# Arthur151/ROMP

Measured on AMD Instinct MI355X. Metric: images/sec (512x512, HRNet-32), higher is better.
Workload: dtype f32 (convs as f16x2-split products, f32 accumulate; same 1e-4 parity gate as f32 MFMA); 1 GPU; ROMP HRNet-32 512x512, batch=1024 synthetic images sharded across 1 GPU (BASELINE configs[2]), each shard walked in forward calls of batch=32 (BASELINE configs[1]); net+parse+SMPL per call; batch_per_call=32, global_batch=1024, hipgraph=True, autotune=True, variant_table=committed romp_amd/tune/romp_hrnet32_f16x2_b32.json, branch_streams=True, conv_math=f16x2, parallelism=dp1, cross_step_pipeline=True, rccl_ranks=1, backend=none (single process)

## Files before the change

### __graft_entry__.py

```python
import os
import sys

ROOT = os.path.dirname(os.path.abspath(__file__))
if ROOT not in sys.path:
    sys.path.insert(0, ROOT)


def build():
    import subprocess
    from romp_amd import build as b
    path = b.build(force=False)
    assert os.path.exists(path)
    import romp_amd
    from romp_amd import lib
    h = lib.load()
    for name in lib.EXPORTS + lib.VIEW_EXPORTS:
        assert hasattr(h, name), name
    from oracle import romp_oracle
    if os.path.isdir('/root/reference/simple_romp/vis_human/sim3drender/lib'):
        subprocess.run(['make', '-C', os.path.join(ROOT, 'oracle')], check=True, stdout=subprocess.DEVNULL)
        from oracle import sim3dr_oracle, ref_cpu
        assert sim3dr_oracle.load_ref() is not None
        assert ref_cpu.available() and ref_cpu.bev_available(), 'oracle/_ref/{romp,bev}/*.pyc missing'
    print('built', path, 'abi', h.romp_abi_version())


def smoke():
    import numpy as np
    import torch
    assert torch.cuda.is_available(), 'smoke() needs the MI355X'
    import romp_amd
    from oracle import romp_oracle as O
    settings = romp_amd.romp_settings([])
    settings.GPU, settings.center_thresh, settings.max_batch = 0, 1.3, 2
    sd = O.make_romp_state_dict(0, center_bias=2.0)
    smpl = O.make_synthetic_smpl(0)
    model = romp_amd.ROMP(settings, state_dict=sd, smpl_model=smpl)
    img = O.make_images(1, seed=3)
    out, bids = model.forward_batch(img.to('cuda:0'))
    torch.cuda.synchronize()
    cm, pm = O.romp_net_forward(sd, img)
    ref = O.parsing_outputs(cm.numpy(), pm.numpy(), settings.center_thresh)
    assert out is not None and ref is not None
    assert np.array_equal(out['center_preds'].cpu().numpy(), ref['center_preds']), 'detections differ'
    th = out['smpl_thetas'].cpu().numpy()
    vo, jo, _ = O.smpl_forward(smpl, out['smpl_betas'].cpu().numpy(), th)
    ev = float(np.abs(out['verts'].cpu().numpy() - vo).max())
    et = float(np.abs(th - ref['smpl_thetas']).max())
    print(f'smoke: {len(ref["batch_ids"])} persons, verts max-abs vs oracle {ev:.2e}, thetas {et:.2e}')
    assert ev < 1e-4, ev
    assert et < 1e-3, et


if __name__ == '__main__':
    build()
    if len(sys.argv) > 1 and sys.argv[1] == 'smoke':
        smoke()
```

### romp_amd/build.py

```python
import concurrent.futures as cf
import os
import subprocess
import sys

HERE = os.path.dirname(os.path.abspath(__file__))
CSRC = os.path.join(HERE, 'csrc')
LIB = os.path.join(HERE, 'libromp_hip.so')
SOURCES = ['conv_h2.hip', 'conv_h2c.hip', 'conv_h2c32.hip', 'conv_f32.hip', 'conv_h2d.hip', 'conv_h2b.hip', 'conv_h2r.hip',
           'conv_h2s.hip', 'conv_mfma.hip', 'conv_h2k.hip', 'conv_h2g.hip', 'conv_h2x.hip', 'conv_fup.hip', 'stem_fuse.hip', 'stem2.hip', 'stem7p.hip', 'net.hip', 'parse.hip', 'smpl.hip', 'bev.hip',
           'post.hip', 'crowd.hip', 'render.hip', 'temporal.hip']
OPTIONAL_BX3 = 'conv_bx3.hip'
_UNROLL = ['-mllvm', '-pragma-unroll-threshold=1000000']
EXTRA_FLAGS = {'conv_h2b.hip': _UNROLL, 'conv_h2c.hip': _UNROLL, 'conv_h2c32.hip': _UNROLL}
FLAGS = ['--offload-arch=gfx950', '-O3', '-std=c++17', '-fPIC', '-Wall', '-Wno-unused-function', '-Wno-unused-value', '-Wno-unused-result']


def _hipcc():
    for c in (os.environ.get('HIPCC'), '/opt/rocm/bin/hipcc', 'hipcc'):
        if c and (os.path.isabs(c) and os.path.exists(c) or not os.path.isabs(c)):
            return c
    raise RuntimeError('hipcc not found')


def _stale(target, deps):
    if not os.path.exists(target):
        return True
    t = os.path.getmtime(target)
    return any(os.path.getmtime(d) > t for d in deps)


def build(force=False, verbose=False, extra_flags=(), lib=None, objdir=None, with_bx3=None):
    hipcc = _hipcc()
    if with_bx3 is None:
        with_bx3 = os.environ.get('ROMP_WITH_BX3', '0') not in ('', '0')
    sources = SOURCES + ([OPTIONAL_BX3] if with_bx3 else [])
    headers = [os.path.join(CSRC, f) for f in os.listdir(CSRC) if f.endswith('.h')] + \
              [os.path.join(HERE, '..', 'include', h) for h in ('romp_hip.h', 'romp_hip_views.h')]
    objdir = objdir or os.path.join(HERE, 'build')
    lib = lib or LIB
    os.makedirs(objdir, exist_ok=True)
    jobs = []
    for s in sources:
        src = os.path.join(CSRC, s)
        obj = os.path.join(objdir, s.replace('.hip', '.o'))
        if force or _stale(obj, [src] + headers):
            jobs.append((src, obj))

    def cc(job):
        src, obj = job
        cmd = [hipcc] + FLAGS + list(extra_flags) + EXTRA_FLAGS.get(os.path.basename(src), []) + ['-c', src, '-o', obj]
        r = subprocess.run(cmd, capture_output=True, text=True)
        if r.returncode != 0:
            raise RuntimeError('hipcc failed for %s:\n%s' % (src, r.stderr[-4000:]))
        if verbose and r.stderr.strip():
            print(r.stderr, file=sys.stderr)
        return obj

    with cf.ThreadPoolExecutor(max_workers=min(8, max(1, len(jobs)))) as ex:
        list(ex.map(cc, jobs))
    objs = [os.path.join(objdir, s.replace('.hip', '.o')) for s in sources]
    marker = os.path.join(objdir, '.with_bx3')
    relink = os.path.exists(marker) != bool(with_bx3)
    if force or jobs or relink or _stale(lib, objs):
        cmd = [hipcc, '--offload-arch=gfx950', '-shared', '-fPIC'] + objs + ['-o', lib]
        r = subprocess.run(cmd, capture_output=True, text=True)
        if r.returncode != 0:
            raise RuntimeError('link failed:\n' + r.stderr[-4000:])
        if with_bx3:
            open(marker, 'w').close()
        elif os.path.exists(marker):
            os.remove(marker)
    return lib


if __name__ == '__main__':
    print(build(force='--force' in sys.argv, verbose=True))
```

### romp_amd/csrc/common.h

```cpp
#pragma once
#include <hip/hip_runtime.h>
#include <stdint.h>
#include <stdio.h>
#include <stdarg.h>
#include "../../include/romp_hip.h"

namespace romp {

void set_error(const char* fmt, ...);

#define ROMP_HIP_CHECK(expr)                                                          \
    do {                                                                              \
        hipError_t _e = (expr);                                                       \
        if (_e != hipSuccess) {                                                       \
            romp::set_error("%s failed: %s (%s:%d)", #expr, hipGetErrorString(_e),    \
                            __FILE__, __LINE__);                                      \
            return ROMP_EHIP;                                                         \
        }                                                                             \
    } while (0)

#define ROMP_REQUIRE(cond, ...)                                                       \
    do {                                                                              \
        if (!(cond)) {                                                                \
            romp::set_error(__VA_ARGS__);                                             \
            return ROMP_EINVAL;                                                       \
        }                                                                             \
    } while (0)

constexpr int QUEUE_STRIDE = 32, QUEUE_INTS = 8 * QUEUE_STRIDE;

int launch_conv(const romp_op& op, const float* in, const float* res, float* out, int B,
                int mode, int variant, int* queue, hipStream_t st, int wg_cap = 0);
int describe_conv(const romp_op& op, int B, int variant, char* out, int n);
int conv_num_variants();
int conv_family_variants(int math);
int conv_trace_read(unsigned long long* dst_host, int max_words);
int conv_init();
bool conv_variant_valid(const romp_op& op, int variant);
bool conv_variant_tunable(const romp_op& op, int variant);
void conv_set_sat_counter(int* counter, bool checked_fused);
int* conv_sat_counter();
void conv_set_wg_cap(int cap);
int conv_wg_cap();
bool conv_sat_checked();
unsigned long long* conv_trace_arm(hipStream_t st);
int launch_seam1x1(const romp_op& opa, const romp_op& opb, const romp_op* opd, const float* m, const float* x, float* t, float* u, int B, hipStream_t st);
int launch_bblock32r(const romp_op& op1, const romp_op& op2, const float* x, float* y, int B, int* queue, hipStream_t st);
int launch_bblock64(const romp_op& op1, const romp_op& op2, const float* x, float* y, int B, int* queue, hipStream_t st);
int launch_bblock32(const romp_op& op1, const romp_op& op2, const float* x, float* y, int B, int* queue, hipStream_t st);
int launch_stem(const romp_op& op, const float* image, float* out, int B, hipStream_t st);
int launch_stem7(const romp_op& op, const float* image, float* out, int B, hipStream_t st);
int launch_stem2(const romp_op& stem, const romp_op& op, const float* image, float* out, int B, hipStream_t st);
int launch_maxpool(const romp_op& op, const float* in, float* out, int B, hipStream_t st);
int launch_stem7p(const romp_op& op, const float* image, float* out, int B, hipStream_t st);
struct FuseTerm { const float* ptr; int shift; int cstride; int fmt; };
int launch_fusesum(const FuseTerm* terms, int n_terms, float* out, int B, int H, int W, int C,
                   int out_cstride, int out_coff, int relu, hipStream_t st, int out_fmt = 0, int act_shift = 0);

int launch_fuseup(const romp_op& op, const FuseTerm* terms, float* out, int B, hipStream_t st);

int launch_ksum(const romp_op& op, const float* partial, const float* res, float* out, int B, hipStream_t st);

int launch_bev_pack(const float* fv, int fv_cs, const float* feats, int f_cs, float* out, int B, hipStream_t st);
int launch_bev_maps(const float* fv, int fv_cs, const float* bv, int bv_cs, const float* anchors_host, float* center3d,
                    float* cam3d, int B, hipStream_t st);
int launch_conv3d(int C, const float* w_host, const float* scale_host, const float* shift_host, int relu, const float* in,
                  const float* res, float* out, int B, hipStream_t st);

}
```

### romp_amd/csrc/parse.hip

```cpp
#include "common.h"
#include "rot6d.h"
#include <vector>

#pragma clang fp contract(off)

namespace romp {

constexpr int MAP = 64, NPIX = MAP * MAP;

constexpr int PARSE_THREADS = 1024;
__global__ __launch_bounds__(PARSE_THREADS) void parse_nms_topk_kernel(const float* __restrict__ center, float thresh,
                                                              int max_person, int32_t* __restrict__ ws) {
    __shared__ float s_map[NPIX];
    __shared__ float s_score[NPIX];
    __shared__ int s_idx[NPIX];
    __shared__ int s_count;
    const int b = blockIdx.x, tid = threadIdx.x;
    const float* cm = center + (size_t)b * NPIX;
    for (int p = tid; p < NPIX; p += PARSE_THREADS) s_map[p] = cm[p];
    if (tid == 0) s_count = 0;
    __syncthreads();
    for (int p = tid; p < NPIX; p += PARSE_THREADS) {
        const int y = p / MAP, x = p % MAP;
        const float v = s_map[p];
        float m = v;
        for (int dy = -2; dy <= 2; ++dy) {
            const int yy = y + dy;
            if ((unsigned)yy >= (unsigned)MAP) continue;
            for (int dx = -2; dx <= 2; ++dx) {
                const int xx = x + dx;
                if ((unsigned)xx >= (unsigned)MAP) continue;
                m = fmaxf(m, s_map[yy * MAP + xx]);
            }
        }
        const float score = (m == v) ? v : v * 0.0f;
        if (score > thresh) {
            const int slot = atomicAdd(&s_count, 1);
            s_score[slot] = score;
            s_idx[slot] = p;
        }
    }
    __syncthreads();
    const int n = s_count;
    int32_t* w = ws + (size_t)b * (2 * max_person + 2);
    for (int c = tid; c < n; c += PARSE_THREADS) {
        const float sc = s_score[c];
        const int id = s_idx[c];
        int rank = 0;
        for (int k = 0; k < n; ++k) {
            const float so = s_score[k];
            rank += (so > sc) || (so == sc && s_idx[k] < id);
        }
        if (rank < max_person) {
            w[rank] = id;
            w[max_person + rank] = __float_as_int(sc);
        }
    }
    if (tid == 0) {
        w[2 * max_person] = n < max_person ? n : max_person;
        w[2 * max_person + 1] = n;
    }
}

__global__ __launch_bounds__(64) void parse_pack_kernel(
    const float* __restrict__ center, const float* __restrict__ params, int B, int max_person,
    int32_t* __restrict__ ws, int32_t* batch_ids, int32_t* flat_inds, float* scores, float* params_pred,
    float* cam, float* thetas, float* betas, int32_t* center_preds, const int32_t* watch) {
    const int r = blockIdx.x, b = blockIdx.y, lane = threadIdx.x;
    const int stride = 2 * max_person + 2;
    if (watch && r == 0 && b == 0 && lane == 0)
        ws[(size_t)B * stride] = __hip_atomic_load(watch, __ATOMIC_RELAXED, __HIP_MEMORY_SCOPE_AGENT);
    const int cnt = ws[(size_t)b * stride + 2 * max_person];
    if (r >= cnt) return;
    int off = 0;
    for (int k = lane; k < b; k += 64) off += ws[(size_t)k * stride + 2 * max_person];
    for (int d = 32; d > 0; d >>= 1) off += __shfl_xor(off, d);
    const int row = off + r;
    const int flat = ws[(size_t)b * stride + r];
    const float sc = __int_as_float(ws[(size_t)b * stride + max_person + r]);
    __shared__ float s_p[148];
    const float* src = params + ((size_t)b * NPIX + flat) * 145;
    for (int c = lane; c < 145; c += 64) {
        float v = src[c];
        if (c == 0) v = powf(1.1f, v);
        s_p[c] = v;
        params_pred[(size_t)row * 145 + c] = v;
    }
    __syncthreads();
    if (lane < 3) cam[row * 3 + lane] = s_p[lane];
    if (lane < 10) betas[row * 10 + lane] = s_p[135 + lane];
    if (lane < 22) {
        float aa[3];
        rot6d_to_aa_dev(s_p + 3 + lane * 6, aa);
        thetas[row * 72 + lane * 3 + 0] = aa[0];
        thetas[row * 72 + lane * 3 + 1] = aa[1];
        thetas[row * 72 + lane * 3 + 2] = aa[2];
    } else if (lane < 28) {
        thetas[row * 72 + 66 + (lane - 22)] = 0.f;
    }
    if (lane == 0) {
        batch_ids[row] = b;
        flat_inds[row] = flat;
        scores[row] = sc;
        center_preds[row * 2 + 0] = (flat % MAP) * 512 / 64;
        center_preds[row * 2 + 1] = (flat / MAP) * 512 / 64;
    }
}

__global__ void rot6d_kernel(const float* __restrict__ x6, int n, float* __restrict__ aa) {
    const int i = blockIdx.x * blockDim.x + threadIdx.x;
    if (i >= n) return;
    float x[6], o[3];
    for (int k = 0; k < 6; ++k) x[k] = x6[(size_t)i * 6 + k];
    rot6d_to_aa_dev(x, o);
    for (int k = 0; k < 3; ++k) aa[(size_t)i * 3 + k] = o[k];
}

__global__ void project_kernel(const float* __restrict__ joints, int N, int J, const float* __restrict__ cam,
                               float pad_size, float left, float top, float* pj2d, float* pj2d_org,
                               float* cam_trans) {
    const int i = blockIdx.x * blockDim.x + threadIdx.x;
    if (i < N * J) {
        const int n = i / J;
        const float s = cam[n * 3], tx = cam[n * 3 + 1], ty = cam[n * 3 + 2];
        const float px = joints[(size_t)i * 3] * s + tx, py = joints[(size_t)i * 3 + 1] * s + ty;
        pj2d[(size_t)i * 2] = px; pj2d[(size_t)i * 2 + 1] = py;
        pj2d_org[(size_t)i * 2] = (px + 1.f) * pad_size / 2.f - left;
        pj2d_org[(size_t)i * 2 + 1] = (py + 1.f) * pad_size / 2.f - top;
    }
    if (i < N) {
        const float s = cam[i * 3], tx = cam[i * 3 + 1], ty = cam[i * 3 + 2];
        cam_trans[i * 3 + 0] = (tx / s) * 2.f;
        cam_trans[i * 3 + 1] = (ty / s) * 2.f;
        cam_trans[i * 3 + 2] = (1.f / s) * 2.f;
    }
}

__global__ void cam_to_trans_kernel(const float* __restrict__ cam, int N, float weight, float* __restrict__ trans) {
    const int i = blockIdx.x * blockDim.x + threadIdx.x;
    if (i >= N) return;
    const float s = cam[i * 3], tx = cam[i * 3 + 1], ty = cam[i * 3 + 2];
    trans[i * 3 + 0] = (tx / s) * weight;
    trans[i * 3 + 1] = (ty / s) * weight;
    trans[i * 3 + 2] = (1.f / s) * weight;
}

__global__ __launch_bounds__(64) void translation_lsq_kernel(const float* __restrict__ joints, int J, int K, const float* __restrict__ pj2d,
                                                               double f, double cx, double cy, float* __restrict__ trans) {
    const int n = blockIdx.x, lane = threadIdx.x;
    double a02 = 0, a12 = 0, a22 = 0, b0 = 0, b1 = 0, b2 = 0;
    int cnt = 0;
    for (int k = lane; k < K; k += 64) {
        const float* X = joints + ((size_t)n * J + k) * 3;
        const float uf = (pj2d[((size_t)n * J + k) * 2] + 1.f) * (float)cx, vf = (pj2d[((size_t)n * J + k) * 2 + 1] + 1.f) * (float)cy;
        if (!(vf > -2.f) || X[2] == -2.f) continue;
        ++cnt;
        const double u = uf, v = vf;
        const double qx = cx - u, qy = cy - v;
        const double rx = (u - cx) * (double)X[2] - f * (double)X[0], ry = (v - cy) * (double)X[2] - f * (double)X[1];
        a02 += f * qx; a12 += f * qy; a22 += qx * qx + qy * qy;
        b0 += f * rx; b1 += f * ry; b2 += qx * rx + qy * ry;
    }
    for (int d = 32; d > 0; d >>= 1) {
        a02 += __shfl_xor(a02, d); a12 += __shfl_xor(a12, d); a22 += __shfl_xor(a22, d);
        b0 += __shfl_xor(b0, d); b1 += __shfl_xor(b1, d); b2 += __shfl_xor(b2, d);
        cnt += __shfl_xor(cnt, d);
    }
    if (lane == 0) {
        const double d = (double)cnt * f * f;
        const double piv = a22 - (a02 * a02 + a12 * a12) / d;
        float t0 = -1.f, t1 = -1.f, t2 = -1.f;
        if (cnt >= 4 && fabs(piv) > 1e-12 * fabs(a22)) {
            const double z = (b2 - (a02 * b0 + a12 * b1) / d) / piv;
            t0 = (float)((b0 - a02 * z) / d); t1 = (float)((b1 - a12 * z) / d); t2 = (float)z;
        }
        trans[n * 3] = t0; trans[n * 3 + 1] = t1; trans[n * 3 + 2] = t2;
    }
}

#pragma clang fp contract(off)
__global__ void project_verts_kernel(const float* __restrict__ verts, size_t total, int V, const float* __restrict__ cam,
                                     float pad_size, float left, float top, float* __restrict__ camed, float* __restrict__ org) {
    const size_t i = blockIdx.x * (size_t)blockDim.x + threadIdx.x;
    if (i >= total) return;
    const size_t n = i / V;
    const float s = cam[n * 3], tx = cam[n * 3 + 1], ty = cam[n * 3 + 2];
    const float px = verts[i * 3] * s + tx, py = verts[i * 3 + 1] * s + ty, pz = verts[i * 3 + 2];
    if (camed) { camed[i * 3] = px; camed[i * 3 + 1] = py; camed[i * 3 + 2] = pz; }
    org[i * 3] = (px + 1.f) * pad_size / 2.f - left;
    org[i * 3 + 1] = (py + 1.f) * pad_size / 2.f - top;
    org[i * 3 + 2] = (pz + 1.f) * pad_size / 2.f;
}

__global__ void bev_project_verts_kernel(const float* __restrict__ verts, size_t total, int V, const float* __restrict__ trans,
                                         float pad_size, float left, float top, float* __restrict__ org) {
    const size_t i = blockIdx.x * (size_t)blockDim.x + threadIdx.x;
    if (i >= total) return;
    const size_t n = i / V;
    const float vz = verts[i * 3 + 2];
    const float x = verts[i * 3] + trans[n * 3], y = verts[i * 3 + 1] + trans[n * 3 + 1], z = vz + trans[n * 3 + 2] + 1e-6f;
    const float px = x / z * 443.4f / 256.f, py = y / z * 443.4f / 256.f;
    org[i * 3] = (px + 1.f) * pad_size / 2.f - left;
    org[i * 3 + 1] = (py + 1.f) * pad_size / 2.f - top;
    org[i * 3 + 2] = (vz + 1.f) * pad_size / 2.f;
}

}

using namespace romp;

extern "C" {

int romp_bev_project_verts(const float* verts, int N, int V, const float* cam_trans, const float* pad_info_host, float* verts_camed_org,
                           void* stream) {
    ROMP_REQUIRE(verts && cam_trans && pad_info_host && verts_camed_org && N > 0 && V > 0, "romp_bev_project_verts: bad arguments");
    const float top = pad_info_host[0], left = pad_info_host[2], h = pad_info_host[4], w = pad_info_host[5];
    const size_t total = (size_t)N * V;
    hipLaunchKernelGGL(bev_project_verts_kernel, dim3((unsigned)((total + 255) / 256)), dim3(256), 0, (hipStream_t)stream, verts, total,
                       V, cam_trans, h > w ? h : w, left, top, verts_camed_org);
    ROMP_HIP_CHECK(hipGetLastError());
    return ROMP_OK;
}

int romp_project_verts(const float* verts, int N, int V, const float* cam, const float* pad_info_host, float* verts_camed,
                       float* verts_camed_org, void* stream) {
    ROMP_REQUIRE(verts && cam && pad_info_host && verts_camed_org && N > 0 && V > 0, "romp_project_verts: bad arguments");
    const float top = pad_info_host[0], left = pad_info_host[2], h = pad_info_host[4], w = pad_info_host[5];
    const size_t total = (size_t)N * V;
    hipLaunchKernelGGL(project_verts_kernel, dim3((unsigned)((total + 255) / 256)), dim3(256), 0, (hipStream_t)stream, verts, total, V,
                       cam, h > w ? h : w, left, top, verts_camed, verts_camed_org);
    ROMP_HIP_CHECK(hipGetLastError());
    return ROMP_OK;
}

int romp_parse_watch(const float* center_maps, const float* params_maps, int B, float conf_thresh, int max_person,
                     int32_t* count_host, int32_t* batch_ids, int32_t* flat_inds, float* scores, float* params_pred,
                     float* cam, float* thetas, float* betas, int32_t* center_preds, int32_t* workspace, void* stream,
                     const int32_t* watch, int32_t* watch_host) {
    ROMP_REQUIRE(center_maps && params_maps && workspace && B > 0, "romp_parse: bad arguments");
    ROMP_REQUIRE(max_person >= 1 && max_person <= 1024, "romp_parse: max_person %d out of range", max_person);
    ROMP_REQUIRE(batch_ids && flat_inds && scores && params_pred && cam && thetas && betas && center_preds,
                 "romp_parse: null output");
    hipStream_t st = (hipStream_t)stream;
    hipLaunchKernelGGL(parse_nms_topk_kernel, dim3(B), dim3(PARSE_THREADS), 0, st, center_maps, conf_thresh, max_person, workspace);
    ROMP_HIP_CHECK(hipGetLastError());
    hipLaunchKernelGGL(parse_pack_kernel, dim3(max_person, B), dim3(64), 0, st, center_maps, params_maps, B, max_person,
                       workspace, batch_ids, flat_inds, scores, params_pred, cam, thetas, betas, center_preds, watch);
    ROMP_HIP_CHECK(hipGetLastError());
    if (!count_host) return ROMP_OK;
    const size_t n_cnt = (size_t)B * (2 * max_person + 2);
    std::vector<int32_t> cnt(n_cnt + 1);
    ROMP_HIP_CHECK(hipMemcpyAsync(cnt.data(), workspace, (n_cnt + (watch ? 1 : 0)) * sizeof(int32_t), hipMemcpyDeviceToHost, st));
    ROMP_HIP_CHECK(hipStreamSynchronize(st));
    int total = 0;
    for (int b = 0; b < B; ++b) total += cnt[(size_t)b * (2 * max_person + 2) + 2 * max_person];
    *count_host = total;
    if (watch && watch_host) *watch_host = cnt[n_cnt];
    return ROMP_OK;
}

int romp_parse(const float* center_maps, const float* params_maps, int B, float conf_thresh, int max_person,
               int32_t* count_host, int32_t* batch_ids, int32_t* flat_inds, float* scores, float* params_pred,
               float* cam, float* thetas, float* betas, int32_t* center_preds, int32_t* workspace, void* stream) {
    return romp_parse_watch(center_maps, params_maps, B, conf_thresh, max_person, count_host, batch_ids, flat_inds, scores, params_pred,
                            cam, thetas, betas, center_preds, workspace, stream, nullptr, nullptr);
}

int romp_rot6d_to_aa(const float* x6, int n, float* aa, void* stream) {
    ROMP_REQUIRE(x6 && aa && n >= 0, "romp_rot6d_to_aa: bad arguments");
    if (n == 0) return ROMP_OK;
    hipLaunchKernelGGL(rot6d_kernel, dim3((n + 127) / 128), dim3(128), 0, (hipStream_t)stream, x6, n, aa);
    ROMP_HIP_CHECK(hipGetLastError());
    return ROMP_OK;
}

int romp_cam_to_trans(const float* cam, int N, float weight, float* trans, void* stream) {
    ROMP_REQUIRE(cam && trans && N >= 0, "romp_cam_to_trans: bad arguments");
    if (N == 0) return ROMP_OK;
    hipLaunchKernelGGL(cam_to_trans_kernel, dim3((N + 255) / 256), dim3(256), 0, (hipStream_t)stream, cam, N, weight, trans);
    ROMP_HIP_CHECK(hipGetLastError());
    return ROMP_OK;
}

int romp_estimate_translation(const float* joints, int N, int J, int K, const float* pj2d, float focal_length, float img_size,
                              float* trans, void* stream) {
    ROMP_REQUIRE(joints && pj2d && trans && N >= 0 && J > 0 && K >= 2 && K <= J, "romp_estimate_translation: bad arguments");
    if (N == 0) return ROMP_OK;
    hipLaunchKernelGGL(translation_lsq_kernel, dim3(N), dim3(64), 0, (hipStream_t)stream, joints, J, K, pj2d, (double)focal_length,
                       (double)img_size / 2.0, (double)img_size / 2.0, trans);
    ROMP_HIP_CHECK(hipGetLastError());
    return ROMP_OK;
}

int romp_project(const float* joints, int N, int J, const float* cam, const float* pad_info_host, float* pj2d,
                 float* pj2d_org, float* cam_trans, void* stream) {
    ROMP_REQUIRE(joints && cam && pad_info_host && pj2d && pj2d_org && cam_trans && N >= 0 && J > 0,
                 "romp_project: bad arguments");
    if (N == 0) return ROMP_OK;
    const float top = pad_info_host[0], left = pad_info_host[2], h = pad_info_host[4], w = pad_info_host[5];
    const float pad_size = h > w ? h : w;
    const int total = N * J;
    hipLaunchKernelGGL(project_kernel, dim3((total + 255) / 256), dim3(256), 0, (hipStream_t)stream, joints, N, J, cam,
                       pad_size, left, top, pj2d, pj2d_org, cam_trans);
    ROMP_HIP_CHECK(hipGetLastError());
    return ROMP_OK;
}

}
```

### romp_amd/csrc/smpl.hip

```cpp
#include "common.h"
#include <vector>

namespace romp {

constexpr int NV = 6890, NJ = 24, NPF = 207, NJOUT = 71, NREG = 26, NPICK = 21;
constexpr int PB = 16;
constexpr int NT = (NV + 63) / 64;
constexpr int MAXLV = NJ;

typedef float f2 __attribute__((ext_vector_type(2)));
__device__ __forceinline__ f2 pk_fma(f2 a, f2 b, f2 c) { return __builtin_elementwise_fma(a, b, c); }

struct Parents { int p[NJ]; };
struct Levels { int n; int start[MAXLV + 1]; int order[NJ]; };

__global__ __launch_bounds__(256) void smpl_prep_kernel(const float* __restrict__ Jreg, const float* __restrict__ vt,
                                                         const float* __restrict__ sd, int nb, float* __restrict__ Jt,
                                                         float* __restrict__ Js) {
    const int j = blockIdx.x, e = blockIdx.y;
    const int k = e / (nb + 1), l = e % (nb + 1);
    double acc = 0.0;
    for (int v = threadIdx.x; v < NV; v += 256) {
        const float w = Jreg[(size_t)j * NV + v];
        const float x = (l == nb) ? vt[v * 3 + k] : sd[((size_t)v * 3 + k) * nb + l];
        acc += (double)w * (double)x;
    }
    __shared__ double s[256];
    s[threadIdx.x] = acc;
    __syncthreads();
    for (int d = 128; d > 0; d >>= 1) {
        if (threadIdx.x < d) s[threadIdx.x] += s[threadIdx.x + d];
        __syncthreads();
    }
    if (threadIdx.x == 0) {
        if (l == nb) Jt[j * 3 + k] = (float)s[0];
        else Js[(j * 3 + k) * nb + l] = (float)s[0];
    }
}

template <int NB>
__global__ __launch_bounds__(64) void smpl_pose_kernel(const float* __restrict__ betas,
                                                        const float* __restrict__ thetas,
                                                        const float* __restrict__ Jt, const float* __restrict__ Js,
                                                        const int* __restrict__ sched, float* __restrict__ pose_feat,
                                                        float* __restrict__ Amat, float* __restrict__ joints) {
    __shared__ float sR[NJ][9], sJ[NJ][3], sG[NJ][12];
    const int n = blockIdx.x, lane = threadIdx.x;
    if (lane < NJ) {
        const float* r = thetas + (size_t)n * 72 + lane * 3;
        const float rx0 = r[0], ry0 = r[1], rz0 = r[2];
        float jt[3], js[3][NB], bt[NB];
#pragma unroll
        for (int l = 0; l < NB; ++l) bt[l] = betas[(size_t)n * NB + l];
#pragma unroll
        for (int k = 0; k < 3; ++k) {
            jt[k] = Jt[lane * 3 + k];
#pragma unroll
            for (int l = 0; l < NB; ++l) js[k][l] = Js[(lane * 3 + k) * NB + l];
        }
        const float ex = rx0 + 1e-8f, ey = ry0 + 1e-8f, ez = rz0 + 1e-8f;
        const float angle = sqrtf(ex * ex + ey * ey + ez * ez);
        const float rx = rx0 / angle, ry = ry0 / angle, rz = rz0 / angle;
        float sn, cs;
        sincosf(angle, &sn, &cs);
        const float oc = 1.f - cs;
        const float kk00 = -(rz * rz) - ry * ry, kk11 = -(rz * rz) - rx * rx, kk22 = -(ry * ry) - rx * rx;
        const float kk01 = ry * rx, kk02 = rz * rx, kk12 = rz * ry;
        float R[9];
        R[0] = 1.f + oc * kk00;      R[1] = sn * -rz + oc * kk01; R[2] = sn * ry + oc * kk02;
        R[3] = sn * rz + oc * kk01;  R[4] = 1.f + oc * kk11;      R[5] = sn * -rx + oc * kk12;
        R[6] = sn * -ry + oc * kk02; R[7] = sn * rx + oc * kk12;  R[8] = 1.f + oc * kk22;
#pragma unroll
        for (int e = 0; e < 9; ++e) sR[lane][e] = R[e];
        if (lane >= 1) {
            float* pf = pose_feat + (size_t)(n / PB) * NPF * PB + (n % PB);
#pragma unroll
            for (int e = 0; e < 9; ++e) pf[((lane - 1) * 9 + e) * PB] = R[e] - ((e == 0 || e == 4 || e == 8) ? 1.f : 0.f);
        }
#pragma unroll
        for (int k = 0; k < 3; ++k) {
            float a = jt[k];
#pragma unroll
            for (int l = 0; l < NB; ++l) a = fmaf(bt[l], js[k][l], a);
            sJ[lane][k] = a;
        }
    }
    __syncthreads();
    const int grp = lane / 12, el = lane % 12, rr = el / 4, cc = el % 4;
    if (lane < 12) sG[0][lane] = (cc < 3) ? sR[0][rr * 3 + cc] : sJ[0][rr];
    __syncthreads();
    const int n_lv = sched[0];
    for (int lv = 1; lv < n_lv; ++lv) {
        const int q1 = sched[1 + lv + 1];
        for (int q = sched[1 + lv] + grp; q < q1 && grp < 5; q += 5) {
            const int i = sched[1 + (MAXLV + 1) + q], p = sched[1 + (MAXLV + 1) + NJ + i];
            float v;
            if (cc < 3) {
                v = sG[p][rr * 4 + 0] * sR[i][0 * 3 + cc];
                v = fmaf(sG[p][rr * 4 + 1], sR[i][1 * 3 + cc], v);
                v = fmaf(sG[p][rr * 4 + 2], sR[i][2 * 3 + cc], v);
            } else {
                v = sG[p][rr * 4 + 0] * (sJ[i][0] - sJ[p][0]);
                v = fmaf(sG[p][rr * 4 + 1], sJ[i][1] - sJ[p][1], v);
                v = fmaf(sG[p][rr * 4 + 2], sJ[i][2] - sJ[p][2], v);
                v += sG[p][rr * 4 + 3];
            }
            sG[i][el] = v;
        }
        __syncthreads();
    }
    for (int idx = lane; idx < NJ * 12; idx += 64) {
        const int j = idx / 12, e = idx % 12, r = e / 4, c = e % 4;
        float v = sG[j][e];
        if (c == 3) {
            joints[((size_t)n * NJOUT + j) * 3 + r] = v;
            const float t = sG[j][r * 4 + 0] * sJ[j][0] + sG[j][r * 4 + 1] * sJ[j][1] + sG[j][r * 4 + 2] * sJ[j][2];
            v -= t;
        }
        Amat[(size_t)n * NJ * 12 + idx] = v;
    }
}

constexpr int SKIN_WAVES = 4, KQ = (NPF + SKIN_WAVES - 1) / SKIN_WAVES;
constexpr int PPW = PB / SKIN_WAVES;
constexpr int U_FLOATS = SKIN_WAVES * PB * 3 * 64;
constexpr int KC = 13, NCH = KQ / KC;
static_assert(KQ == KC * NCH, "chunking of the pose-blend quarter");

__device__ __forceinline__ void pd_load(float (&d)[KC][3], const float* __restrict__ pdv, int kbase) {
#pragma unroll
    for (int i = 0; i < KC; ++i) {
        const size_t off = (size_t)min(kbase + i, NPF - 1) * (NV * 3);
        d[i][0] = pdv[off]; d[i][1] = pdv[off + 1]; d[i][2] = pdv[off + 2];
    }
}

__device__ __forceinline__ void pd_blend(f2 (&po)[PB / 2][3], const float (&d)[KC][3], const float (*s_pf)[PB], int kbase) {
#pragma unroll
    for (int i = 0; i < KC; ++i) {
        const int k = kbase + i;
        const bool in = k < NPF;
        const float d0 = in ? d[i][0] : 0.f, d1 = in ? d[i][1] : 0.f, d2 = in ? d[i][2] : 0.f;
        const f2 dd0{d0, d0}, dd1{d1, d1}, dd2{d2, d2};
        const float* row = s_pf[min(k, NPF - 1)];
#pragma unroll
        for (int p4 = 0; p4 < PB; p4 += 4) {
            const float4 f = *reinterpret_cast<const float4*>(row + p4);
            const f2 fa{f.x, f.y}, fb{f.z, f.w};
            po[p4 / 2][0] = pk_fma(fa, dd0, po[p4 / 2][0]); po[p4 / 2][1] = pk_fma(fa, dd1, po[p4 / 2][1]); po[p4 / 2][2] = pk_fma(fa, dd2, po[p4 / 2][2]);
            po[p4 / 2 + 1][0] = pk_fma(fb, dd0, po[p4 / 2 + 1][0]); po[p4 / 2 + 1][1] = pk_fma(fb, dd1, po[p4 / 2 + 1][1]); po[p4 / 2 + 1][2] = pk_fma(fb, dd2, po[p4 / 2 + 1][2]);
        }
    }
}

constexpr int SVS = 196, RS = 68;
constexpr int RPAIRS = NREG / 2;
static_assert(NREG % 2 == 0 && PB * RPAIRS <= 256, "joint partials: one pass");
template <int NB>
__global__ __launch_bounds__(256) void smpl_skin_kernel(const float* __restrict__ betas, const float* __restrict__ pose_feat,
                                                         const float* __restrict__ Amat, const float* __restrict__ vt,
                                                         const float* __restrict__ sd, const float* __restrict__ pd,
                                                         const float* __restrict__ lbsw, const float* __restrict__ reg, int N, int groups,
                                                         float* __restrict__ verts, float* __restrict__ jpart) {
    __shared__ __attribute__((aligned(16))) float s_u[U_FLOATS];
    __shared__ __attribute__((aligned(16))) float s_A[5 * 256 * 4];
    __shared__ float s_beta[PB][NB];
    static_assert(NPF * PB <= U_FLOATS && 4 * 256 * 4 <= U_FLOATS && PB * SVS <= U_FLOATS && NREG * RS <= PB * NJ * 12 && NT % 4 == 0, "LDS aliasing");
    const int tid = threadIdx.x, lane = tid & 63, wave = tid >> 6;
    const int xcd = blockIdx.x & 7, slot = blockIdx.x >> 3;
    const int tile = (slot / groups) * 8 + xcd, grp = slot % groups;
    if (tile >= NT) return;
    const int p0 = grp * PB;
    const int np = min(PB, N - p0);
    const bool live = tile * 64 + lane < NV;
    const int v = min(tile * 64 + lane, NV - 1);
    const float* pdv = pd + (size_t)v * 3;
    const int k0 = wave * KQ;
    float d[2][KC][3];
    pd_load(d[0], pdv, k0);
    constexpr int PF4 = NPF * PB / 4, A4 = PB * NJ * 12 / 4;
    static_assert(PF4 <= 4 * 256 && A4 <= 5 * 256 && PB * NB <= 256, "staging loops");
    const float4* src_pf = reinterpret_cast<const float4*>(pose_feat + (size_t)grp * NPF * PB);
    const float4* src_A = reinterpret_cast<const float4*>(Amat + (size_t)p0 * NJ * 12);
    float4 tpf[4], tA[5];
#pragma unroll
    for (int i = 0; i < 4; ++i) tpf[i] = src_pf[min(tid + 256 * i, PF4 - 1)];
#pragma unroll
    for (int i = 0; i < 5; ++i) tA[i] = src_A[min(tid + 256 * i, A4 - 1)];
    const float tb = (tid < PB * NB && tid / NB < np) ? betas[(size_t)p0 * NB + tid] : 0.f;
#pragma unroll
    for (int i = 0; i < 4; ++i) reinterpret_cast<float4*>(s_u)[tid + 256 * i] = tpf[i];
#pragma unroll
    for (int i = 0; i < 5; ++i) reinterpret_cast<float4*>(s_A)[tid + 256 * i] = tA[i];
    if (tid < PB * NB) (&s_beta[0][0])[tid] = tb;
    __syncthreads();
    const float(*s_pf)[PB] = reinterpret_cast<const float(*)[PB]>(s_u);
    f2 po[PB / 2][3];
#pragma unroll
    for (int p = 0; p < PB / 2; ++p) po[p][0] = po[p][1] = po[p][2] = f2{0.f, 0.f};
#pragma unroll
    for (int c = 0; c < NCH; ++c) {
        if (c + 1 < NCH) pd_load(d[(c + 1) & 1], pdv, k0 + (c + 1) * KC);
        pd_blend(po, d[c & 1], s_pf, k0 + c * KC);
    }
    const float t0 = vt[v * 3 + 0], t1 = vt[v * 3 + 1], t2 = vt[v * 3 + 2];
    float sdv[3][NB];
#pragma unroll
    for (int k = 0; k < 3; ++k)
#pragma unroll
        for (int l = 0; l < NB; ++l) sdv[k][l] = sd[((size_t)v * 3 + k) * NB + l];
    f2 w[NJ];
#pragma unroll
    for (int j4 = 0; j4 < NJ; j4 += 4) {
        const float4 t = *reinterpret_cast<const float4*>(lbsw + (size_t)v * NJ + j4);
        w[j4] = f2{t.x, t.x}; w[j4 + 1] = f2{t.y, t.y}; w[j4 + 2] = f2{t.z, t.z}; w[j4 + 3] = f2{t.w, t.w};
    }
    float treg[7];
    static_assert(NREG * 64 <= 7 * 256, "regressor tile staging");
#pragma unroll
    for (int i = 0; i < 7; ++i) {
        const int idx = min(tid + 256 * i, NREG * 64 - 1), vv = tile * 64 + (idx & 63);
        const float x = reg[(size_t)(idx >> 6) * NV + min(vv, NV - 1)];
        treg[i] = vv < NV ? x : 0.f;
    }
    __syncthreads();
    float(*s_po)[PB * 3][64] = reinterpret_cast<float(*)[PB * 3][64]>(s_u);
#pragma unroll
    for (int p = 0; p < PB / 2; ++p)
#pragma unroll
        for (int k = 0; k < 3; ++k) {
            s_po[wave][(2 * p) * 3 + k][lane] = po[p][k].x;
            s_po[wave][(2 * p + 1) * 3 + k][lane] = po[p][k].y;
        }
    __syncthreads();
    float out[PPW][3];
#pragma unroll
    for (int pp = 0; pp < PPW; ++pp) {
        const int p = wave * PPW + pp;
        float a0 = 0.f, a1 = 0.f, a2 = 0.f;
#pragma unroll
        for (int l = 0; l < NB; ++l) {
            const float bb = s_beta[p][l];
            a0 = fmaf(bb, sdv[0][l], a0); a1 = fmaf(bb, sdv[1][l], a1); a2 = fmaf(bb, sdv[2][l], a2);
        }
        float q[3];
#pragma unroll
        for (int k = 0; k < 3; ++k)
            q[k] = (s_po[0][p * 3 + k][lane] + s_po[1][p * 3 + k][lane]) + (s_po[2][p * 3 + k][lane] + s_po[3][p * 3 + k][lane]);
        const float x = q[0] + (t0 + a0), y = q[1] + (t1 + a1), z = q[2] + (t2 + a2);
        f2 T[6];
#pragma unroll
        for (int e = 0; e < 6; ++e) T[e] = f2{0.f, 0.f};
        const float* Ap = s_A + p * NJ * 12;
#pragma unroll
        for (int j = 0; j < NJ; ++j) {
            const float4 a0v = *reinterpret_cast<const float4*>(Ap + j * 12);
            const float4 a1v = *reinterpret_cast<const float4*>(Ap + j * 12 + 4);
            const float4 a2v = *reinterpret_cast<const float4*>(Ap + j * 12 + 8);
            T[0] = pk_fma(w[j], f2{a0v.x, a0v.y}, T[0]); T[1] = pk_fma(w[j], f2{a0v.z, a0v.w}, T[1]);
            T[2] = pk_fma(w[j], f2{a1v.x, a1v.y}, T[2]); T[3] = pk_fma(w[j], f2{a1v.z, a1v.w}, T[3]);
            T[4] = pk_fma(w[j], f2{a2v.x, a2v.y}, T[4]); T[5] = pk_fma(w[j], f2{a2v.z, a2v.w}, T[5]);
        }
        out[pp][0] = fmaf(T[0].x, x, fmaf(T[0].y, y, fmaf(T[1].x, z, T[1].y)));
        out[pp][1] = fmaf(T[2].x, x, fmaf(T[2].y, y, fmaf(T[3].x, z, T[3].y)));
        out[pp][2] = fmaf(T[4].x, x, fmaf(T[4].y, y, fmaf(T[5].x, z, T[5].y)));
        if (live && p < np) {
            float* o = verts + ((size_t)(p0 + p) * NV + v) * 3;
            o[0] = out[pp][0]; o[1] = out[pp][1]; o[2] = out[pp][2];
        }
    }
    __syncthreads();
#pragma unroll
    for (int pp = 0; pp < PPW; ++pp)
#pragma unroll
        for (int k = 0; k < 3; ++k) s_u[(wave * PPW + pp) * SVS + k * 64 + lane] = out[pp][k];
#pragma unroll
    for (int i = 0; i < 7; ++i) {
        const int idx = tid + 256 * i;
        if (idx < NREG * 64) s_A[(idx >> 6) * RS + (idx & 63)] = treg[i];
    }
    __syncthreads();
    if (tid < PB * RPAIRS) {
        const int p = tid % PB, rp = tid / PB;
        const float* sv = s_u + p * SVS;
        const float* sr = s_A + rp * 2 * RS;
        f2 acc[3] = {f2{0.f, 0.f}, f2{0.f, 0.f}, f2{0.f, 0.f}};
#pragma unroll 4
        for (int i = 0; i < 64; i += 4) {
            const float4 x4 = *reinterpret_cast<const float4*>(sv + i), y4 = *reinterpret_cast<const float4*>(sv + 64 + i),
                         z4 = *reinterpret_cast<const float4*>(sv + 128 + i);
            const float4 r0 = *reinterpret_cast<const float4*>(sr + i), r1 = *reinterpret_cast<const float4*>(sr + RS + i);
#define JSTEP(c)                                                             \
            acc[0] = pk_fma(f2{r0.c, r1.c}, f2{x4.c, x4.c}, acc[0]);        \
            acc[1] = pk_fma(f2{r0.c, r1.c}, f2{y4.c, y4.c}, acc[1]);        \
            acc[2] = pk_fma(f2{r0.c, r1.c}, f2{z4.c, z4.c}, acc[2]);
            JSTEP(x) JSTEP(y) JSTEP(z) JSTEP(w)
#undef JSTEP
        }
        if (p < np) {
            float* o = jpart + (((size_t)(p0 + p) * NT + tile) * NREG + rp * 2) * 3;
            o[0] = acc[0].x; o[1] = acc[1].x; o[2] = acc[2].x;
            o[3] = acc[0].y; o[4] = acc[1].y; o[5] = acc[2].y;
        }
    }
}

__global__ __launch_bounds__(256) void smpl_joints_kernel(const float* __restrict__ verts, const float* __restrict__ jpart,
                                                           const int* __restrict__ pick, int root_align, float* __restrict__ joints,
                                                           float* __restrict__ root) {
    __shared__ float s_j[NJOUT * 3];
    const int n = blockIdx.x, tid = threadIdx.x;
    const float* vn = verts + (size_t)n * NV * 3;
    float* jn = joints + (size_t)n * NJOUT * 3;
    __shared__ float s_part[3][NREG * 3];
    static_assert(NT % 3 == 0 && 3 * NREG * 3 <= 256 && NREG * 3 + NPICK * 3 + NJ * 3 <= 256, "thread roles");
    if (tid < 3 * NREG * 3) {
        const int e = tid % (NREG * 3), part = tid / (NREG * 3);
        const float* src = jpart + ((size_t)n * NT + part * (NT / 3)) * NREG * 3 + e;
        float t[NT / 3];
#pragma unroll
        for (int u = 0; u < NT / 3; ++u) t[u] = src[(size_t)u * NREG * 3];
        float acc[4] = {0.f, 0.f, 0.f, 0.f};
#pragma unroll
        for (int u = 0; u < NT / 3; ++u) acc[u & 3] += t[u];
        s_part[part][e] = (acc[0] + acc[1]) + (acc[2] + acc[3]);
    }
    __syncthreads();
    if (tid < NREG * 3) {
        s_j[(NJ + NPICK) * 3 + tid] = (s_part[0][tid] + s_part[1][tid]) + s_part[2][tid];
    } else if (tid < NREG * 3 + NPICK * 3) {
        const int e = tid - NREG * 3;
        s_j[NJ * 3 + e] = vn[pick[e / 3] * 3 + e % 3];
    } else if (tid < NREG * 3 + NPICK * 3 + NJ * 3) {
        const int e = tid - NREG * 3 - NPICK * 3;
        s_j[e] = jn[e];
    }
    __syncthreads();
    if (tid < NJOUT * 3) {
        float v = s_j[tid];
        if (root_align) {
            const float r0 = (s_j[45 * 3 + tid % 3] + s_j[46 * 3 + tid % 3]) / 2.f;
            v -= r0;
            if (tid < 3) root[n * 3 + tid] = r0;
        }
        if (root_align || tid >= NJ * 3) jn[tid] = v;
    }
}

__global__ __launch_bounds__(256) void smpl_root_sub_kernel(float* __restrict__ verts, const float* __restrict__ root) {
    const int n = blockIdx.y, i = blockIdx.x * 256 + threadIdx.x;
    static_assert(NV * 3 % 2 == 0, "person stride is a whole number of float2");
    if (i >= NV * 3 / 2) return;
    const float r0 = root[n * 3], r1 = root[n * 3 + 1], r2 = root[n * 3 + 2];
    float2* p = reinterpret_cast<float2*>(verts + (size_t)n * NV * 3) + i;
    float2 t = *p;
    const int c = (i * 2) % 3;
    t.x -= c == 0 ? r0 : (c == 1 ? r1 : r2);
    t.y -= c == 0 ? r1 : (c == 1 ? r2 : r0);
    *p = t;
}

}

using namespace romp;

struct smpl_ctx {
    int nb = 10;
    int cap = 0;
    Parents par;
    int* sched = nullptr;
    float* jpart = nullptr;
    float *vt = nullptr, *sd = nullptr, *pd = nullptr, *lbsw = nullptr, *reg = nullptr, *Jt = nullptr, *Js = nullptr;
    int* pick = nullptr;
    float *pose_feat = nullptr, *Amat = nullptr, *root = nullptr;
};

static int smpl_reserve(smpl_ctx* c, int N, hipStream_t st) {
    if (N <= c->cap) return ROMP_OK;
    if (c->pose_feat) hipFree(c->pose_feat);
    if (c->Amat) hipFree(c->Amat);
    if (c->root) hipFree(c->root);
    if (c->jpart) hipFree(c->jpart);
    c->pose_feat = c->Amat = c->root = c->jpart = nullptr;
    c->cap = 0;
    const size_t cap = (size_t)(N + PB - 1) / PB * PB;
    ROMP_HIP_CHECK(hipMalloc((void**)&c->pose_feat, cap * NPF * 4));
    ROMP_HIP_CHECK(hipMalloc((void**)&c->Amat, cap * NJ * 12 * 4));
    ROMP_HIP_CHECK(hipMalloc((void**)&c->root, cap * 3 * 4));
    ROMP_HIP_CHECK(hipMalloc((void**)&c->jpart, cap * NT * NREG * 3 * 4));
    ROMP_HIP_CHECK(hipMemsetAsync(c->pose_feat, 0, cap * NPF * 4, st));
    ROMP_HIP_CHECK(hipMemsetAsync(c->Amat, 0, cap * NJ * 12 * 4, st));
    c->cap = (int)cap;
    return ROMP_OK;
}

extern "C" {

int smpl_ctx_create(smpl_ctx** out, const float* v_template, const float* shapedirs, int n_betas,
                    const float* posedirs, const float* J_regressor, const float* lbs_weights,
                    const int64_t* parents_host, const float* J_regressor_extra9, const float* J_regressor_h36m17,
                    const int64_t* extra_idx_host, int max_persons, void* stream) {
    ROMP_REQUIRE(out && v_template && shapedirs && posedirs && J_regressor && lbs_weights && parents_host &&
                 J_regressor_extra9 && J_regressor_h36m17 && extra_idx_host, "smpl_ctx_create: null argument");
    ROMP_REQUIRE(n_betas == 10 || n_betas == 11, "smpl_ctx_create: n_betas %d (10 = SMPL, 11 = SMPL-A)", n_betas);
    hipStream_t st = (hipStream_t)stream;
    smpl_ctx* c = new smpl_ctx();
    c->nb = n_betas;
    for (int j = 0; j < NJ; ++j) {
        c->par.p[j] = (int)parents_host[j];
        if (j > 0 && (c->par.p[j] < 0 || c->par.p[j] >= j)) {
            set_error("smpl_ctx_create: parents[%d]=%d is not an earlier joint", j, c->par.p[j]);
            delete c;
            return ROMP_EINVAL;
        }
    }
    int sched_h[1 + (MAXLV + 1) + 2 * NJ] = {0}, depth[NJ] = {0}, n_lv = 1;
    for (int j = 1; j < NJ; ++j) {
        depth[j] = depth[c->par.p[j]] + 1;
        if (depth[j] + 1 > n_lv) n_lv = depth[j] + 1;
    }
    sched_h[0] = n_lv;
    for (int lv = 0, q = 0; lv < n_lv; ++lv) {
        sched_h[1 + lv] = q;
        for (int j = 0; j < NJ; ++j)
            if (depth[j] == lv) sched_h[1 + (MAXLV + 1) + q++] = j;
        sched_h[1 + lv + 1] = q;
    }
    for (int j = 0; j < NJ; ++j) sched_h[1 + (MAXLV + 1) + NJ + j] = j ? c->par.p[j] : 0;
    int pick_h[NPICK];
    for (int i = 0; i < NPICK; ++i) {
        pick_h[i] = (int)extra_idx_host[i];
        if (pick_h[i] < 0 || pick_h[i] >= NV) { set_error("smpl_ctx_create: extra index out of range"); delete c; return ROMP_EINVAL; }
    }
#define SMPL_ALLOC_COPY(dst, src, count)                                                           \
    do {                                                                                           \
        if (hipMalloc((void**)&(dst), (size_t)(count) * 4) != hipSuccess ||                        \
            hipMemcpyAsync((dst), (src), (size_t)(count) * 4, hipMemcpyDeviceToDevice, st) != hipSuccess) { \
            set_error("smpl_ctx_create: alloc/copy of " #dst " failed");                           \
            smpl_ctx_destroy(c);                                                                   \
            return ROMP_EHIP;                                                                      \
        }                                                                                          \
    } while (0)
    SMPL_ALLOC_COPY(c->vt, v_template, NV * 3);
    SMPL_ALLOC_COPY(c->sd, shapedirs, (size_t)NV * 3 * n_betas);
    SMPL_ALLOC_COPY(c->pd, posedirs, (size_t)NPF * NV * 3);
    SMPL_ALLOC_COPY(c->lbsw, lbs_weights, (size_t)NV * NJ);
#undef SMPL_ALLOC_COPY
    if (hipMalloc((void**)&c->reg, (size_t)NREG * NV * 4) != hipSuccess || hipMalloc((void**)&c->Jt, NJ * 3 * 4) != hipSuccess ||
        hipMalloc((void**)&c->Js, (size_t)NJ * 3 * n_betas * 4) != hipSuccess || hipMalloc((void**)&c->pick, NPICK * 4) != hipSuccess ||
        hipMalloc((void**)&c->sched, sizeof(sched_h)) != hipSuccess) {
        set_error("smpl_ctx_create: hipMalloc failed");
        smpl_ctx_destroy(c);
        return ROMP_ENOMEM;
    }
    hipMemcpyAsync(c->reg, J_regressor_extra9, (size_t)9 * NV * 4, hipMemcpyDeviceToDevice, st);
    hipMemcpyAsync(c->reg + (size_t)9 * NV, J_regressor_h36m17, (size_t)17 * NV * 4, hipMemcpyDeviceToDevice, st);
    hipMemcpyAsync(c->pick, pick_h, NPICK * 4, hipMemcpyHostToDevice, st);
    hipMemcpyAsync(c->sched, sched_h, sizeof(sched_h), hipMemcpyHostToDevice, st);
    hipLaunchKernelGGL(smpl_prep_kernel, dim3(NJ, 3 * (n_betas + 1)), dim3(256), 0, st, J_regressor, c->vt, c->sd, n_betas,
                       c->Jt, c->Js);
    if (hipStreamSynchronize(st) != hipSuccess || hipGetLastError() != hipSuccess) {
        set_error("smpl_ctx_create: constant preparation failed");
        smpl_ctx_destroy(c);
        return ROMP_EHIP;
    }
    int rc = smpl_reserve(c, max_persons > 0 ? max_persons : 64, st);
    if (rc) { smpl_ctx_destroy(c); return rc; }
    if (hipStreamSynchronize(st) != hipSuccess) {
        set_error("smpl_ctx_create: clearing the staging buffers failed");
        smpl_ctx_destroy(c);
        return ROMP_EHIP;
    }
    *out = c;
    return ROMP_OK;
}

int smpl_forward(smpl_ctx* c, const float* betas, int n_betas, const float* thetas, int N, int root_align,
                 float* verts, float* joints, void* stream) {
    ROMP_REQUIRE(c && betas && thetas && verts && joints && N >= 0, "smpl_forward: bad arguments");
    ROMP_REQUIRE(n_betas == c->nb, "smpl_forward: n_betas %d but context was built with %d", n_betas, c->nb);
    if (N == 0) return ROMP_OK;
    hipStream_t st = (hipStream_t)stream;
    int rc = smpl_reserve(c, N, st);
    if (rc) return rc;
    if (c->nb == 10)
        hipLaunchKernelGGL(smpl_pose_kernel<10>, dim3(N), dim3(64), 0, st, betas, thetas, c->Jt, c->Js, c->sched, c->pose_feat, c->Amat, joints);
    else
        hipLaunchKernelGGL(smpl_pose_kernel<11>, dim3(N), dim3(64), 0, st, betas, thetas, c->Jt, c->Js, c->sched, c->pose_feat, c->Amat, joints);
    ROMP_HIP_CHECK(hipGetLastError());
    const int groups = (N + PB - 1) / PB;
    const dim3 grid(8 * ((NT + 7) / 8) * groups);
    if (c->nb == 10)
        hipLaunchKernelGGL(smpl_skin_kernel<10>, grid, dim3(256), 0, st, betas, c->pose_feat, c->Amat, c->vt, c->sd, c->pd,
                           c->lbsw, c->reg, N, groups, verts, c->jpart);
    else
        hipLaunchKernelGGL(smpl_skin_kernel<11>, grid, dim3(256), 0, st, betas, c->pose_feat, c->Amat, c->vt, c->sd, c->pd,
                           c->lbsw, c->reg, N, groups, verts, c->jpart);
    ROMP_HIP_CHECK(hipGetLastError());
    hipLaunchKernelGGL(smpl_joints_kernel, dim3(N), dim3(256), 0, st, verts, c->jpart, c->pick, root_align, joints, c->root);
    ROMP_HIP_CHECK(hipGetLastError());
    if (root_align) {
        hipLaunchKernelGGL(smpl_root_sub_kernel, dim3((NV * 3 / 2 + 255) / 256, N), dim3(256), 0, st, verts, c->root);
        ROMP_HIP_CHECK(hipGetLastError());
    }
    return ROMP_OK;
}

void smpl_ctx_destroy(smpl_ctx* c) {
    if (!c) return;
    float* ptrs[] = {c->vt, c->sd, c->pd, c->lbsw, c->reg, c->Jt, c->Js, c->pose_feat, c->Amat, c->root, c->jpart};
    for (float* p : ptrs)
        if (p) hipFree(p);
    if (c->pick) hipFree(c->pick);
    if (c->sched) hipFree(c->sched);
    delete c;
}

}
```

### romp_amd/distributed.py

```python
import torch
import torch.distributed as dist

RECORD_BASE = 88


def shard_range(n_items, rank, world_size):
    base, rem = divmod(n_items, world_size)
    lo = rank * base + min(rank, rem)
    return lo, lo + base + (1 if rank < rem else 0)


def pack_records(outputs, batch_ids, img_offset, flat_inds=None, with_joints=False, with_verts=False):
    if outputs is None:
        return None
    N = outputs['cam'].shape[0]
    dev = outputs['cam'].device
    flat = flat_inds if flat_inds is not None else (outputs['center_preds'][:, 1] // 8 * 64 + outputs['center_preds'][:, 0] // 8)
    cols = [(batch_ids + img_offset).float().view(N, 1), flat.float().view(N, 1), outputs['center_confs'].view(N, 1),
            outputs['cam'], outputs['smpl_thetas'], outputs['smpl_betas']]
    if with_joints:
        cols.append(outputs['joints'].reshape(N, -1))
    if with_verts:
        cols.append(outputs['verts'].reshape(N, -1))
    return torch.cat([c.to(dev).float() for c in cols], 1).contiguous()


def record_width(with_joints=False, with_verts=False):
    return RECORD_BASE + (213 if with_joints else 0) + (6890 * 3 if with_verts else 0)


def all_gather_records(local, width, device, group=None, state=None):
    world = dist.get_world_size(group)
    n_local = 0 if local is None else local.shape[0]
    if state is not None and state.get('cap', 0) > 0:
        cap = state['cap']
        block = torch.zeros(cap + 1, width, device=device, dtype=torch.float32)
        block[0, 0] = float(n_local)
        if n_local:
            block[1:1 + min(n_local, cap)] = local[:cap]
        gathered = torch.empty(world * (cap + 1), width, device=device, dtype=torch.float32)
        _all_gather_block(gathered, block, world, device, group)
        counts = [int(v) for v in gathered.view(world, cap + 1, width)[:, 0, 0].tolist()]
        if max(counts) <= cap:
            state['exchanges'] = state.get('exchanges', 0) + 1
            parts = [gathered[r * (cap + 1) + 1: r * (cap + 1) + 1 + counts[r]] for r in range(world)]
            return (torch.cat(parts, 0) if sum(counts) else torch.zeros(0, width, device=device)), counts
        state['cap'] = _capacity(max(counts))
        state['regrown'] = state.get('regrown', 0) + 1
        return all_gather_records(local, width, device, group, state)
    counts = [torch.zeros(1, dtype=torch.int64, device=device) for _ in range(world)]
    dist.all_gather(counts, torch.tensor([n_local], dtype=torch.int64, device=device), group=group)
    counts = torch.cat(counts).tolist()
    n_max = max(counts)
    if state is not None:
        state['cap'] = _capacity(n_max)
    if n_max == 0:
        return torch.zeros(0, width, device=device), counts
    block = torch.zeros(n_max, width, device=device, dtype=torch.float32)
    if n_local:
        block[:n_local] = local
    gathered = torch.empty(world * n_max, width, device=device, dtype=torch.float32)
    _all_gather_block(gathered, block, world, device, group)
    parts = [gathered[r * n_max: r * n_max + counts[r]] for r in range(world)]
    return torch.cat(parts, 0), counts


def _capacity(n_max):
    return max(64, -(-int(n_max) * 5 // 4))


def _all_gather_block(gathered, block, world, device, group):
    if device.type == 'cuda' and hasattr(dist, 'all_gather_into_tensor'):
        dist.all_gather_into_tensor(gathered, block, group=group)
    else:
        _all_gather_list(gathered, block, world, group)


def _all_gather_list(gathered, block, world, group):
    outs = list(gathered.chunk(world, 0))
    dist.all_gather(outs, block, group=group)


def unpack_records(rec, with_joints=False, with_verts=False):
    out = {
        'image_ids': rec[:, 0].long(), 'flat_inds': rec[:, 1].long(), 'center_confs': rec[:, 2:3],
        'cam': rec[:, 3:6], 'smpl_thetas': rec[:, 6:78], 'smpl_betas': rec[:, 78:88],
    }
    o = RECORD_BASE
    if with_joints:
        out['joints'] = rec[:, o:o + 213].reshape(-1, 71, 3)
        o += 213
    if with_verts:
        out['verts'] = rec[:, o:o + 6890 * 3].reshape(-1, 6890, 3)
    return out


def local_records(model, images_local, img_offset, chunk=None, with_joints=True, with_verts=False, next_images=None):
    n = images_local.shape[0]
    chunk = n if not chunk else int(chunk)
    recs = []
    if chunk < n and hasattr(model, 'forward_chunks'):
        it = model.forward_chunks(images_local, chunk, next_images=next_images) if next_images is not None else model.forward_chunks(images_local, chunk)
    else:
        it = ((*model.forward_batch(images_local[c0:c0 + chunk]), c0) for c0 in range(0, n, chunk))
    for outputs, batch_ids, c0 in it:
        r = pack_records(outputs, batch_ids, img_offset + c0, with_joints=with_joints, with_verts=with_verts)
        if r is not None:
            recs.append(r)
    if not recs:
        return None
    return recs[0] if len(recs) == 1 else torch.cat(recs, 0)


def sharded_forward(model, images_local, img_offset, with_joints=True, with_verts=False, group=None, chunk=None, next_images=None,
                    gather_state=None):
    dev = images_local.device
    rec = local_records(model, images_local, img_offset, chunk, with_joints, with_verts, next_images=next_images)
    allrec, counts = all_gather_records(rec, record_width(with_joints, with_verts), dev, group, gather_state)
    return unpack_records(allrec, with_joints, with_verts), counts
```

### romp_amd/lib.py

```python
import ctypes as C
import os

_HERE = os.path.dirname(os.path.abspath(__file__))
LIB_PATH = os.environ.get('ROMP_HIP_LIB') or os.path.join(_HERE, 'libromp_hip.so')

ABI_VERSION = 7
BUF_NONE, BUF_IMAGE, BUF_CENTER, BUF_PARAMS = -1, -2, -3, -4
FMT_F32, FMT_H2 = 0, 1
OP_STEM, OP_CONV, OP_FUSESUM, OP_FORK, OP_JOIN, OP_BEV_PACK, OP_BEV_MAPS, OP_CONV3D = 1, 2, 3, 4, 5, 6, 7, 8
OP_NOP, OP_BBLOCK32, OP_BBLOCK64, OP_SEAM1X1, OP_FUSEUP, OP_RECORD, OP_WAIT = 12, 13, 14, 15, 16, 17, 18
OP_KSUM = 11
OP_STEM2 = 19
OP_STEM7, OP_MAXPOOL, OP_STEM7P = 9, 10, 20
OPF_WAVE16, OPF_STEM_VALU, OPF_SEAM_DS = 1, 2, 4


class RompOp(C.Structure):
    _fields_ = [
        ('kind', C.c_int32),
        ('in_buf', C.c_int32), ('out_buf', C.c_int32), ('res_buf', C.c_int32),
        ('H', C.c_int32), ('W', C.c_int32),
        ('Cin', C.c_int32), ('Cout', C.c_int32),
        ('ksize', C.c_int32), ('stride', C.c_int32), ('relu', C.c_int32),
        ('groups', C.c_int32),
        ('in_cstride', C.c_int32), ('in_coff', C.c_int32), ('in_gstride', C.c_int32),
        ('out_cstride', C.c_int32), ('out_coff', C.c_int32), ('out_gstride', C.c_int32),
        ('res_cstride', C.c_int32), ('res_coff', C.c_int32), ('res_gstride', C.c_int32),
        ('cin_pad', C.c_int32), ('cout_pad', C.c_int32),
        ('n_terms', C.c_int32),
        ('term_buf', C.c_int32 * 4), ('term_shift', C.c_int32 * 4), ('term_cstride', C.c_int32 * 4),
        ('stream', C.c_int32), ('pad_h', C.c_int32), ('pad_w', C.c_int32), ('out_rstride', C.c_int32), ('out_bstride', C.c_int32),
        ('in_fmt', C.c_int32), ('out_fmt', C.c_int32), ('res_fmt', C.c_int32), ('term_fmt', C.c_int32 * 4),
        ('act_shift', C.c_int32),
        ('flags', C.c_int32), ('relu_from', C.c_int32), ('term_coff', C.c_int32 * 4),
        ('weight', C.c_void_p), ('scale', C.c_void_p), ('shift', C.c_void_p), ('weight_aux', C.c_void_p),
        ('weight_h2', C.c_void_p), ('scale_h2', C.c_void_p),
    ]


_lib = None


class RompHipError(RuntimeError):
    pass


def load():
    global _lib
    if _lib is not None:
        return _lib
    import torch
    if not os.path.exists(LIB_PATH):
        from . import build as _build
        _build.build()
    lib = C.CDLL(LIB_PATH)
    vp, i32, i64p, f = C.c_void_p, C.c_int, C.POINTER(C.c_int64), C.c_float
    sigs = {
        'romp_abi_version': (C.c_int, []),
        'romp_last_error': (C.c_char_p, []),
        'romp_net_create': (C.c_int, [C.POINTER(vp), C.POINTER(RompOp), i32, i64p, i32, i32]),
        'romp_net_forward': (C.c_int, [vp, vp, i32, vp, vp, vp]),
        'romp_net_read_buffer': (C.c_int, [vp, i32, i32, vp, C.c_int64, vp]),
        'romp_net_write_buffer': (C.c_int, [vp, i32, vp, C.c_int64, vp]),
        'romp_net_set_mode': (C.c_int, [vp, i32]),
        'romp_net_set_graph': (C.c_int, [vp, i32]),
        'romp_net_set_streams': (C.c_int, [vp, i32]),
        'romp_net_profile': (C.c_int, [vp, vp, i32, vp, vp, vp, C.POINTER(C.c_float), i32]),
        'romp_net_range_scan': (C.c_int, [vp, vp, i32, vp, vp, vp, C.POINTER(C.c_float), C.POINTER(C.c_int32), C.POINTER(C.c_int32)]),
        'romp_net_saturated': (C.c_int, [vp, C.POINTER(C.c_int64), i32, vp]),
        'romp_net_set_sat_check': (C.c_int, [vp, i32]),
        'romp_net_destroy': (None, [vp]),
        'romp_conv_forward': (C.c_int, [C.POINTER(RompOp), vp, vp, vp, i32, i32, i32, vp]),
        'romp_conv_num_variants': (C.c_int, []),
        'romp_conv_family_variants': (C.c_int, [i32]),
        'romp_conv_trace_read': (C.c_int, [C.POINTER(C.c_uint64), i32]),
        'romp_conv_describe': (C.c_int, [C.POINTER(RompOp), i32, i32, C.c_char_p, i32]),
        'romp_net_autotune': (C.c_int, [vp, i32, i32, vp]),
        'romp_net_tuned_variant': (C.c_int, [vp, i32, i32]),
        'romp_oneeuro_state_floats': (C.c_int, [i32]),
        'romp_oneeuro_smooth': (C.c_int, [vp, vp, i32, i32, f, vp, vp, vp, vp]),
        'romp_cam_to_trans': (C.c_int, [vp, i32, f, vp, vp]),
        'romp_estimate_translation': (C.c_int, [vp, i32, i32, i32, vp, f, f, vp, vp]),
        'romp_project_verts': (C.c_int, [vp, i32, i32, vp, C.POINTER(C.c_float), vp, vp, vp]),
        'romp_bev_project_verts': (C.c_int, [vp, i32, i32, vp, C.POINTER(C.c_float), vp, vp]),
        'romp_sim3dr_normals': (C.c_int, [vp, vp, vp, vp, i32, vp, vp]),
        'romp_sim3dr_light': (C.c_int, [vp, vp, i32, C.POINTER(C.c_float), vp, vp]),
        'romp_sim3dr_rasterize': (C.c_int, [vp, vp, vp, vp, i32, i32, i32, i32, i32, vp, vp]),
        'romp_sim3dr_render_batch': (C.c_int, [vp, i32, i32, vp, i32, i32, vp, i32, vp, vp, vp, C.POINTER(C.c_float), vp, vp, vp, vp]),
        'romp_view_weak_perspective': (C.c_int, [vp, i32, i32, C.c_double, C.c_double, i32, i32, C.c_double, vp, vp, vp, vp]),
        'romp_net_load': (C.c_int, [C.POINTER(C.c_void_p), C.c_char_p, i32]),
        'romp_net_plan_info': (C.c_int, [vp, C.POINTER(C.c_int32), C.POINTER(C.c_int64), C.POINTER(C.c_int64), C.POINTER(C.c_int32)]),
        'romp_net_plan_kind': (C.c_int, [vp, C.POINTER(C.c_int32)]),
        'romp_net_set_split': (C.c_int, [vp, i32, i32, C.c_int64, C.c_int64, C.c_int64]),
        'romp_net_set_tuned': (C.c_int, [vp, i32, C.POINTER(C.c_int32), i32]),
        'romp_bev_workspace_ints': (C.c_int, [i32, i32]),
        'romp_bev_parse': (C.c_int, [vp, i32, f, i32, C.POINTER(C.c_int32), vp, vp, vp, vp, vp]),
        'romp_bev_regress': (C.c_int, [vp, vp, i32, i32, vp, vp, C.POINTER(C.c_float)] + [vp] * 7 + [vp] * 6 + [vp]),
        'romp_net_buffer_ptr': (C.c_void_p, [vp, i32]),
        'romp_parse': (C.c_int, [vp, vp, i32, f, i32, C.POINTER(C.c_int32), vp, vp, vp, vp, vp, vp, vp, vp, vp, vp]),
        'romp_parse_watch': (C.c_int, [vp, vp, i32, f, i32, C.POINTER(C.c_int32), vp, vp, vp, vp, vp, vp, vp, vp, vp, vp, vp, C.POINTER(C.c_int32)]),
        'romp_net_sat_counter': (C.c_void_p, [vp]),
        'romp_rot6d_to_aa': (C.c_int, [vp, i32, vp, vp]),
        'smpl_ctx_create': (C.c_int, [C.POINTER(vp), vp, vp, i32, vp, vp, vp, i64p, vp, vp, i64p, i32, vp]),
        'smpl_forward': (C.c_int, [vp, vp, i32, vp, i32, i32, vp, vp, vp]),
        'smpl_ctx_destroy': (None, [vp]),
        'romp_preprocess': (C.c_int, [vp, i32, i32, vp, i32, C.POINTER(C.c_float), vp]),
        'romp_preprocess_batch': (C.c_int, [vp, i32, i32, i32, vp, i32, C.POINTER(C.c_float), vp]),
        'romp_bev_postprocess': (C.c_int, [vp, vp, vp, i32, vp, f, f, vp, vp, vp, vp, vp]),
        'romp_project': (C.c_int, [vp, i32, i32, vp, C.POINTER(C.c_float), vp, vp, vp, vp]),
        'romp_preprocess_crops': (C.c_int, [vp, i32, i32, i32, i32, C.POINTER(C.c_int32), vp, i32, C.POINTER(C.c_float), vp]),
        'romp_bev_crowd_merge': (C.c_int, [vp, vp, vp, vp, i32, i32, i32, C.POINTER(C.c_int32), i32, i32, i32, C.c_double, f,
                                           vp, vp, vp, vp, vp, vp]),
    }
    lib.romp_abi_version.restype = C.c_int
    if lib.romp_abi_version() != ABI_VERSION:
        raise RompHipError('%s is ABI version %d, this binding needs %d: rebuild it (python -m romp_amd.build --force)'
                           % (LIB_PATH, lib.romp_abi_version(), ABI_VERSION))
    for name, (res, args) in sigs.items():
        fn = getattr(lib, name)
        fn.restype = res
        fn.argtypes = args

    _lib = lib
    return lib


EXPORTS = ['romp_abi_version', 'romp_last_error', 'romp_net_create', 'romp_net_forward', 'romp_net_read_buffer',
           'romp_net_write_buffer', 'romp_net_set_mode', 'romp_net_set_graph', 'romp_net_set_streams', 'romp_net_profile', 'romp_net_range_scan', 'romp_net_saturated', 'romp_net_set_sat_check', 'romp_net_destroy',
           'romp_conv_forward', 'romp_conv_num_variants', 'romp_conv_family_variants', 'romp_conv_trace_read', 'romp_conv_describe',
           'romp_net_load', 'romp_net_plan_info', 'romp_net_plan_kind', 'romp_net_autotune', 'romp_net_tuned_variant', 'romp_net_set_tuned', 'romp_net_set_split', 'romp_project_verts', 'romp_estimate_translation', 'romp_cam_to_trans', 'romp_bev_project_verts', 'romp_oneeuro_state_floats', 'romp_oneeuro_smooth', 'romp_sim3dr_normals', 'romp_sim3dr_light', 'romp_sim3dr_rasterize', 'romp_bev_workspace_ints', 'romp_bev_parse', 'romp_bev_regress',
           'romp_net_buffer_ptr', 'romp_parse', 'romp_parse_watch', 'romp_net_sat_counter', 'romp_rot6d_to_aa', 'smpl_ctx_create', 'smpl_forward', 'smpl_ctx_destroy',
           'romp_project', 'romp_preprocess', 'romp_preprocess_batch', 'romp_bev_postprocess', 'romp_preprocess_crops',
           'romp_bev_crowd_merge']
VIEW_EXPORTS = ['romp_sim3dr_render_batch', 'romp_view_weak_perspective']


def has_bf16x3():
    h = load()
    return h.romp_conv_family_variants(1) + h.romp_conv_family_variants(2) > 0


def check(rc):
    if rc != 0:
        msg = load().romp_last_error()
        raise RompHipError('libromp_hip error %d: %s' % (rc, msg.decode() if msg else '?'))


def ptr(t):
    return C.c_void_p(0 if t is None else t.data_ptr())


def stream_ptr(device=None):
    import torch
    return C.c_void_p(torch.cuda.current_stream(device).cuda_stream)
```

### romp_amd/main.py

```python
import argparse
import os
import os.path as osp
import sys

import numpy as np
import torch
from torch import nn

from . import lib as L
from .net import RangeGuard, RompNet
from .post_parser import (_HAVE_CV2, CenterMap, SMPL_parser, body_mesh_projection2image, convert_cam_to_3d_trans, pnp_translation,
                          parsing_outputs)
from .vis import rendering_romp_bev_results, setup_renderer
from .utils import ResultSaver, convert_tensor2numpy, determine_device, img_preprocess, img_preprocess_device


def romp_settings(input_args=sys.argv[1:]):
    parser = argparse.ArgumentParser(description='ROMP: Monocular, One-stage, Regression of Multiple 3D People')
    parser.add_argument('-m', '--mode', type=str, default='image', help='Inferece mode, including image, video, webcam')
    parser.add_argument('-i', '--input', type=str, default=None, help='Path to the input image / video')
    parser.add_argument('-o', '--save_path', type=str, default=osp.join(osp.expanduser("~"), 'ROMP_results'), help='Path to save the results')
    parser.add_argument('--GPU', type=int, default=0, help='The gpu device number to run the inference on.')
    parser.add_argument('--onnx', action='store_true', help='(reference flag; the HIP path replaces the ONNX session)')
    parser.add_argument('-t', '--temporal_optimize', action='store_true', help='Whether to use OneEuro filter to smooth the results')
    parser.add_argument('--center_thresh', type=float, default=0.25, help='The confidence threshold of positive detection in 2D human body center heatmap.')
    parser.add_argument('--show_largest', action='store_true', help='Whether to show the largest person only')
    parser.add_argument('-sc', '--smooth_coeff', type=float, default=3., help='The smoothness coeff of OneEuro filter, the smaller, the smoother.')
    parser.add_argument('--calc_smpl', action='store_false', help='Whether to calculate the smpl mesh from estimated SMPL parameters')
    parser.add_argument('--render_mesh', action='store_true', help='Whether to render the estimated 3D mesh mesh to image')
    parser.add_argument('--renderer', type=str, default='sim3dr', help='Choose the renderer for visualizaiton')
    parser.add_argument('--show', action='store_true', help='Whether to show the rendered results')
    parser.add_argument('--show_items', type=str, default='mesh',
                        help='The items to visualized: any of mesh, mesh_bird_view, mesh_side_view (panels in that order)')
    parser.add_argument('--save_video', action='store_true', help='Whether to save the video results')
    parser.add_argument('--frame_rate', type=int, default=24, help='The frame_rate of saved video results')
    parser.add_argument('--smpl_path', type=str, default=osp.join(osp.expanduser("~"), '.romp', 'SMPL_NEUTRAL.pth'), help='The path of smpl model file')
    parser.add_argument('--model_path', type=str, default=osp.join(osp.expanduser("~"), '.romp', 'ROMP.pkl'), help='The path of ROMP checkpoint')
    parser.add_argument('--model_onnx_path', type=str, default=osp.join(osp.expanduser("~"), '.romp', 'ROMP.onnx'), help='The path of ROMP onnx checkpoint')
    parser.add_argument('--root_align', type=bool, default=False, help='Please set this config as True to use the ROMP checkpoints trained by yourself.')
    parser.add_argument('--webcam_id', type=int, default=0, help='The Webcam ID.')
    parser.add_argument('--max_batch', type=int, default=32, help='[romp_amd] largest batch forward_batch will be called with')
    parser.add_argument('--conv_math', type=str, default='f16x2', choices=['f32', 'bf16x3', 'f16x2', 'all'],
                        help='[romp_amd] f32: exact-f32 MFMA kernels only; f16x2 (default) / bf16x3 (needs a library built with ROMP_WITH_BX3=1): also offer the f32-accurate split-precision kernels '
                             '(2 fp16 pieces, 3 products / 3 bf16 pieces, 6 products) on the 16-bit matrix pipe, chosen per layer by measurement the first '
                             'time a batch size is seen; all: both families')
    parser.add_argument('--backbone', type=str, default='hrnet32', choices=['hrnet32', 'resnet50'],
                        help='[romp_amd] hrnet32: the simple_romp model (ROMP.pkl); resnet50: the training tree\'s ResNet-50 variant '
                             '(romp/lib/models/resnet_50.py + romp_model.py state_dict)')
    parser.add_argument('--plan_path', type=str, default=None,
                        help='[romp_amd] start from a plan file (python -m romp_amd.export: the lowered network with its packed constants '
                             'and measured kernel tables) instead of --model_path: the counterpart of the reference\'s --onnx / --model_onnx_path')
    parser.add_argument('--no_calibrate', action='store_true',
                        help='[romp_amd] skip the start-up range calibration of the f16x2 kernels (one float32 forward; tensors whose range does '
                             'not fit fp16 pieces stay float32): ranges are then trusted, out-of-range values saturate (RompNet.saturated counts them)')
    parser.add_argument('--calib_dir', type=str, default=None,
                        help='[romp_amd] calibrate on up to 4 images of this directory (pre-processed like inputs) instead of synthetic frames')
    parser.add_argument('--host_preprocess', action='store_true', help='[romp_amd] pad/resize on the host (cv2 / numpy) instead of the device kernel')
    args = parser.parse_args(input_args)
    if not torch.cuda.is_available():
        args.GPU = -1
        args.temporal_optimize = False
    if args.show:
        args.render_mesh = True
    if args.render_mesh or args.show_largest:
        args.calc_smpl = True
    if not os.path.exists(args.smpl_path):
        alt = args.smpl_path.replace('SMPL_NEUTRAL.pth', 'smpl_packed_info.pth')
        if os.path.exists(alt):
            args.smpl_path = alt
    return args


default_settings = romp_settings(input_args=[])


class ROMP(nn.Module):
    def __init__(self, romp_settings, state_dict=None, smpl_model=None):
        super(ROMP, self).__init__()
        self.settings = romp_settings
        if self.settings.GPU == -1:
            raise L.RompHipError('romp_amd is the MI355X path of ROMP: it needs a HIP device (GPU=%d); '
                                 'there is no CPU fallback' % self.settings.GPU)
        self.tdevice = determine_device(self.settings.GPU)
        self._build_model_(state_dict)
        self.range_guard = RangeGuard(self.model)
        self._initilization_(smpl_model)

    def _build_model_(self, state_dict=None):
        if state_dict is None and getattr(self.settings, 'plan_path', None):
            self.model = RompNet.from_plan(self.settings.plan_path, self.tdevice, max_batch=getattr(self.settings, 'max_batch', 32))
            return
        if state_dict is None:
            state_dict = torch.load(self.settings.model_path, map_location='cpu')
        builder = None
        if getattr(self.settings, 'backbone', 'hrnet32') == 'resnet50':
            from .resnet_plan import build_romp_resnet50 as builder
        self.model = RompNet(state_dict, self.tdevice, max_batch=getattr(self.settings, 'max_batch', 32), builder=builder,
                             bf16x3=getattr(self.settings, 'conv_math', 'f16x2'),
                             calibrate=False if getattr(self.settings, 'no_calibrate', False) else None,
                             calib_images=self._calibration_frames())

    def _calibration_frames(self):
        d = getattr(self.settings, 'calib_dir', None)
        if not d:
            return None
        paths = sorted(osp.join(d, f) for f in os.listdir(d) if f.lower().endswith(('.jpg', '.jpeg', '.png', '.bmp'))) if osp.isdir(d) else [d]
        frames = []
        for path in paths[:4]:
            img = _imread_bgr(path)
            if img is not None:
                frames.append(img_preprocess_device(img, self.tdevice)[0])
        if not frames:
            raise L.RompHipError('--calib_dir %s holds no readable image' % d)
        return torch.cat(frames, 0)

    def _initilization_(self, smpl_model=None):
        self.centermap_parser = CenterMap(conf_thresh=self.settings.center_thresh)
        if self.settings.calc_smpl:
            self.smpl_parser = SMPL_parser(smpl_model if smpl_model is not None else self.settings.smpl_path).to(self.tdevice)
        if self.settings.temporal_optimize:
            self.OE_filters = {}
            if not self.settings.show_largest:
                try:
                    from norfair import Tracker
                except ImportError:
                    raise NotImplementedError('multi-person temporal smoothing associates persons with the third-party norfair '
                                              'tracker (main.py:108-116), which is not installed; use --show_largest')
                from .utils import euclidean_distance
                self.tracker = Tracker(distance_function=euclidean_distance, distance_threshold=200)
                self.tracker_initialized = False
        if self.settings.render_mesh:
            self.visualize_items = self.settings.show_items.split(',')
            self.renderer = setup_renderer(name=self.settings.renderer, device=self.tdevice)

    def single_image_forward(self, image):
        if getattr(self.settings, 'host_preprocess', False):
            input_image, image_pad_info = img_preprocess(image)
            input_image = input_image.to(self.tdevice)
        else:
            input_image, image_pad_info = img_preprocess_device(image, self.tdevice)
        center_maps, params_maps = self.model(input_image)
        parsed_results, rerun = parsing_outputs(center_maps, params_maps, self.centermap_parser, guard=self.range_guard, quiet=True)
        if rerun:
            center_maps, params_maps = self._rerun_f32(input_image)
            parsed_results = parsing_outputs(center_maps, params_maps, self.centermap_parser)
        return parsed_results, image_pad_info

    def _rerun_f32(self, images):
        net32 = self.model.f32_twin()
        center, params = net32.forward_nhwc(images)
        self.range_guard.warn(images)
        return center.unsqueeze(1), params

    def temporal_optimization(self, outputs, signal_ID):
        from .temporal import OneEuroBank
        if signal_ID not in self.OE_filters:
            if len(self.OE_filters) > 100:
                self.OE_filters.clear()
            self.OE_filters[signal_ID] = OneEuroBank(self.tdevice, self.settings.smooth_coeff, outputs['smpl_betas'].shape[1])
        bank = self.OE_filters[signal_ID]
        if self.settings.show_largest:
            max_id = int(torch.argmax(outputs['cam'][:, 0]))
            th, be, ca = (outputs[k][max_id:max_id + 1].contiguous().clone() for k in ('smpl_thetas', 'smpl_betas', 'cam'))
            outputs['smpl_thetas'], outputs['smpl_betas'], outputs['cam'] = bank.smooth([0], th, be, ca)
            return outputs
        import numpy as np
        from norfair import Detection
        from .utils import get_tracked_ids
        detections = [Detection(points=cam[[2, 1]] * 512) for cam in outputs['cam'].cpu().numpy()]
        if not self.tracker_initialized:
            for _ in range(8):
                self.tracker.update(detections=detections)
        tracked_objects = self.tracker.update(detections=detections)
        if len(tracked_objects) == 0:
            return outputs
        tracked_ids = get_tracked_ids(detections, tracked_objects)
        th, be, ca = (outputs[k].contiguous() for k in ('smpl_thetas', 'smpl_betas', 'cam'))
        outputs['smpl_thetas'], outputs['smpl_betas'], outputs['cam'] = bank.smooth(tracked_ids, th, be, ca)
        outputs['track_ids'] = np.array(tracked_ids).astype(np.int32)
        return outputs

    def _finish(self, outputs, image_pad_info):
        outputs['cam_trans'] = convert_cam_to_3d_trans(outputs['cam'])
        if self.settings.calc_smpl:
            outputs = self.smpl_parser(outputs, root_align=self.settings.root_align)
            outputs.update(body_mesh_projection2image(outputs['joints'], outputs['cam'],
                                                      vertices=outputs['verts'] if self.settings.render_mesh else None,
                                                      input2org_offsets=image_pad_info))
        return outputs

    def _forward_fast(self, image):
        x, pad = img_preprocess_device(image, self.tdevice)
        center, params = self.model.forward_nhwc(x)
        result, seen = self._fast_from_maps(center, params, pad, self.range_guard.watch)
        if self.range_guard.check(seen):
            c32, p32 = self._rerun_f32(x)
            result, _ = self._fast_from_maps(c32.squeeze(1), p32, pad, None)
        if result is None:
            print('None person detected')
        return result

    def _fast_from_maps(self, center, params, pad, watch):
        import ctypes as C
        import numpy as np
        from . import lib as L
        lib, dev, cap = L.load(), self.tdevice, self.centermap_parser.max_person
        st = getattr(self, '_fast', None)
        if st is None:
            st = self._fast = dict(ibuf=torch.zeros(cap * 4 + 2 * cap + 2 + 2, device=dev, dtype=torch.int32),
                                   fbuf=torch.zeros(cap * (1 + 145 + 3 + 72 + 10), device=dev, dtype=torch.float32))
        ibuf, fbuf = st['ibuf'], st['fbuf']
        views, at = {}, 0
        for key, w in (('scores', 1), ('params_pred', 145), ('cam', 3), ('smpl_thetas', 72), ('smpl_betas', 10)):
            views[key] = fbuf[at:at + cap * w].view(cap, w)
            at += cap * w
        with torch.cuda.device(dev):
            L.check(lib.romp_parse_watch(L.ptr(center), L.ptr(params), 1, float(self.centermap_parser.conf_thresh), cap, None,
                                         L.ptr(ibuf), L.ptr(ibuf[cap:]), L.ptr(views['scores']), L.ptr(views['params_pred']), L.ptr(views['cam']),
                                         L.ptr(views['smpl_thetas']), L.ptr(views['smpl_betas']), L.ptr(ibuf[2 * cap:]), L.ptr(ibuf[4 * cap:]),
                                         L.stream_ptr(dev), C.c_void_p(watch or 0), None))
        verts, joints, _ = self.smpl_parser.smpl_model(views['smpl_betas'], views['smpl_thetas'], root_align=self.settings.root_align)
        proj = body_mesh_projection2image(joints, views['cam'], input2org_offsets=pad, host_pnp=False)
        small = torch.cat([ibuf.view(torch.float32), fbuf, proj['cam_trans'].reshape(-1), joints.reshape(-1), proj['pj2d_org'].reshape(-1),
                           proj['pj2d'].reshape(-1)])
        host = small.cpu().numpy()
        hi = host[:ibuf.numel()].view(np.int32)
        N = int(hi[4 * cap + 2 * cap])
        seen = int(hi[4 * cap + 2 * cap + 2]) if watch else None
        if N == 0:
            return None, seen
        hf = host[ibuf.numel():]
        out, at = {}, 0
        for key, w in (('scores', 1), ('params_pred', 145), ('cam', 3), ('smpl_thetas', 72), ('smpl_betas', 10), ('cam_trans', 3),
                       ('joints', 213), ('pj2d_org', 142), ('pj2d', 142)):
            out[key] = hf[at:at + cap * w].reshape(cap, w)[:N]
            at += cap * w
        if _HAVE_CV2:
            t = pnp_translation(out['joints'].reshape(N, 71, 3)[:, :24], (out['pj2d'].reshape(N, 71, 2)[:, :24] + 1) * 256)
            if t is not None:
                out['cam_trans'] = t
        th = out['smpl_thetas']
        return {'cam': out['cam'], 'global_orient': np.ascontiguousarray(th[:, :3]), 'body_pose': np.ascontiguousarray(th[:, 3:]),
                'smpl_betas': out['smpl_betas'], 'smpl_thetas': th, 'center_preds': hi[2 * cap:4 * cap].reshape(cap, 2)[:N].astype(np.int64),
                'center_confs': out['scores'].reshape(N, 1), 'cam_trans': out['cam_trans'], 'verts': verts[:N].cpu().numpy(),
                'joints': out['joints'].reshape(N, 71, 3), 'pj2d_org': out['pj2d_org'].reshape(N, 71, 2)}, seen

    def forward(self, image, signal_ID=0, **kwargs):
        s = self.settings
        if (getattr(self, 'fast_single', True) and s.calc_smpl and not s.temporal_optimize and not s.render_mesh
                and not getattr(s, 'host_preprocess', False)):
            return self._forward_fast(image)
        outputs, image_pad_info = self.single_image_forward(image)
        if outputs is None:
            return None
        if self.settings.temporal_optimize:
            outputs = self.temporal_optimization(outputs, signal_ID)
        outputs = self._finish(outputs, image_pad_info)
        if self.settings.render_mesh:
            rendering_cfgs = {'mesh_color': 'identity', 'items': self.visualize_items, 'renderer': self.settings.renderer}
            outputs = rendering_romp_bev_results(self.renderer, outputs, image, rendering_cfgs)
        return convert_tensor2numpy(outputs)

    @torch.no_grad()
    def forward_batch(self, images, return_tensors=True):
        center, params = self.model.forward_nhwc(images)
        outputs, batch_ids, rerun = parsing_outputs(center.unsqueeze(1), params, self.centermap_parser, return_batch_ids=True,
                                                    guard=self.range_guard, quiet=True)
        if rerun:
            c32, p32 = self._rerun_f32(images)
            outputs, batch_ids = parsing_outputs(c32, p32, self.centermap_parser, return_batch_ids=True)
        if outputs is None:
            return None, None
        outputs['cam_trans'] = convert_cam_to_3d_trans(outputs['cam'])
        if self.settings.calc_smpl:
            outputs = self.smpl_parser(outputs, root_align=self.settings.root_align)
        if not return_tensors:
            outputs = convert_tensor2numpy(outputs)
        return outputs, batch_ids


    @torch.no_grad()
    def forward_chunks(self, images, chunk, next_images=None):
        dev = self.tdevice
        n = images.shape[0]
        starts = list(range(0, n, chunk))
        if not hasattr(self, '_pipe'):
            two = os.environ.get('ROMP_PIPE_NETS', '1') == '2' and len(starts) > 1 and self.model.max_batch > 2
            nets = [self.model, self.model.twin()] if two else [self.model, self.model]
            streams = [torch.cuda.Stream(dev), torch.cuda.Stream(dev)] if two else [torch.cuda.Stream(dev)] * 2
            self._pipe = dict(nets=nets, streams=streams, bufs={}, ev_net=[torch.cuda.Event(), torch.cuda.Event()],
                              ev_free=[torch.cuda.Event(), torch.cuda.Event()], primed=None)
        P = self._pipe
        cur = torch.cuda.current_stream(dev)

        def bufs(B, par):
            key = (B, par)
            if key not in P['bufs']:
                P['bufs'][key] = (torch.empty((B,) + tuple(self.model.out_shapes[0]), device=dev),
                                  torch.empty((B,) + tuple(self.model.out_shapes[1]), device=dev))
            return P['bufs'][key]

        def launch(x, par):
            c, p_ = bufs(x.shape[0], par)
            st = P['streams'][par]
            st.wait_event(P['ev_free'][par])
            with torch.cuda.stream(st):
                P['nets'][par].forward_nhwc(x, c, p_)
                P['ev_net'][par].record(st)
            return c, p_

        primed, P['primed'] = P['primed'], None
        if primed is not None and (primed['ptr'], primed['shape'], primed['chunk']) == (images.data_ptr(), tuple(images.shape), chunk):
            off, pending = primed['par'], primed['bufs']
        else:
            off = 0
            P['ev_free'][0].record(cur)
            P['ev_free'][1].record(cur)
            for st in set(P['streams']):
                st.wait_stream(cur)
            pending = launch(images[starts[0]:starts[0] + chunk], off)
        for i, c0 in enumerate(starts):
            center, params = pending
            par = (i + off) & 1
            more = i + 1 < len(starts)
            if more:
                pending = launch(images[starts[i + 1]:starts[i + 1] + chunk], par ^ 1)
            elif next_images is not None and next_images.shape[0] > 0:
                P['primed'] = dict(ptr=next_images.data_ptr(), shape=tuple(next_images.shape), chunk=chunk, par=par ^ 1,
                                   bufs=launch(next_images[:chunk], par ^ 1))
            cur.wait_event(P['ev_net'][par])
            self.range_guard.pipelined = more or P['primed'] is not None
            outputs, batch_ids, rerun = parsing_outputs(center.unsqueeze(1), params, self.centermap_parser, return_batch_ids=True,
                                                        guard=self.range_guard, quiet=True)
            self.range_guard.pipelined = False
            if rerun:
                c32, p32 = self._rerun_f32(images[c0:c0 + chunk])
                outputs, batch_ids = parsing_outputs(c32, p32, self.centermap_parser, return_batch_ids=True)
            if outputs is not None:
                outputs['cam_trans'] = convert_cam_to_3d_trans(outputs['cam'])
                if self.settings.calc_smpl:
                    outputs = self.smpl_parser(outputs, root_align=self.settings.root_align)
            P['ev_free'][par].record(cur)
            yield outputs, batch_ids, c0
        if P['primed'] is None:
            for st in set(P['streams']):
                cur.wait_stream(st)


def _imread_bgr(path):
    try:
        import cv2
        return cv2.imread(path)
    except ImportError:
        from PIL import Image
        try:
            return np.ascontiguousarray(np.asarray(Image.open(path).convert('RGB'))[:, :, ::-1])
        except OSError:
            return None


def main():
    args = romp_settings()
    romp = ROMP(args)
    if args.mode == 'image':
        saver = ResultSaver(args.mode, args.save_path)
        image = _imread_bgr(args.input)
        outputs = romp(image)
        saver(outputs, args.input)
    else:
        raise NotImplementedError('mode %s needs OpenCV capture; only --mode image is wired here' % args.mode)


if __name__ == '__main__':
    main()
```

### romp_amd/post_parser.py

```python
import ctypes as C

import numpy as np
import torch
from torch import nn

from . import lib as L
from .smpl import SMPL


class CenterMap(object):

    def __init__(self, conf_thresh):
        self.size = 64
        self.max_person = 64
        self.sigma = 1
        self.conf_thresh = conf_thresh

    def parse_centermap(self, center_maps, params_maps_nhwc=None):
        r, _ = _parse(center_maps, params_maps_nhwc, self.conf_thresh, self.max_person)
        if r is None:
            e = torch.empty(0, device=center_maps.device)
            return e.long(), e.long(), e.reshape(0, 2), e
        yx = torch.stack([(r['flat_inds'] // self.size).float(), (r['flat_inds'] % self.size).float()], 1)
        return r['batch_ids'], r['flat_inds'], yx, r['scores']


def _parse(center_maps, params_maps_nhwc, conf_thresh, max_person, watch=None):
    lib = L.load()
    dev = center_maps.device
    if dev.type != 'cuda':
        raise L.RompHipError('parsing runs on the HIP device only (no CPU fallback)')
    cm = center_maps.reshape(center_maps.shape[0], 64, 64).contiguous().float()
    B = cm.shape[0]
    if params_maps_nhwc is None:
        params_maps_nhwc = torch.zeros(B, 64, 64, 145, device=dev)
    pm = params_maps_nhwc.contiguous()
    assert pm.shape == (B, 64, 64, 145) and pm.dtype == torch.float32
    cap = B * max_person
    ibuf = torch.empty(cap * 4 + B * (2 * max_person + 2) + 2, device=dev, dtype=torch.int32)
    fbuf = torch.empty(cap * (1 + 145 + 3 + 72 + 10), device=dev, dtype=torch.float32)
    out, at = {}, 0
    for key, w in (('scores', 1), ('params_pred', 145), ('cam', 3), ('smpl_thetas', 72), ('smpl_betas', 10)):
        out[key] = fbuf[at:at + cap * w].view(cap, w) if w > 1 else fbuf[at:at + cap]
        at += cap * w
    out['batch_ids'], out['flat_inds'] = ibuf[:cap], ibuf[cap:2 * cap]
    out['center_preds'] = ibuf[2 * cap:4 * cap].view(cap, 2)
    ws = ibuf[4 * cap:]
    n, w = C.c_int32(0), C.c_int32(0)
    with torch.cuda.device(dev):
        L.check(lib.romp_parse_watch(L.ptr(cm), L.ptr(pm), B, float(conf_thresh), int(max_person), C.byref(n),
                                     L.ptr(out['batch_ids']), L.ptr(out['flat_inds']), L.ptr(out['scores']),
                                     L.ptr(out['params_pred']), L.ptr(out['cam']), L.ptr(out['smpl_thetas']),
                                     L.ptr(out['smpl_betas']), L.ptr(out['center_preds']), L.ptr(ws), L.stream_ptr(dev),
                                     C.c_void_p(watch or 0), C.byref(w)))
    N = n.value
    seen = w.value if watch else None
    if N == 0:
        return None, seen
    out = {k: v[:N] for k, v in out.items()}
    il = ibuf[:4 * cap].long()
    out['batch_ids'], out['flat_inds'], out['center_preds'] = il[:N], il[cap:cap + N], il[2 * cap:4 * cap].view(cap, 2)[:N]
    return out, seen


def parsing_outputs(center_maps, params_maps, centermap_parser, return_batch_ids=False, guard=None, quiet=False):
    if params_maps.dim() == 4 and params_maps.shape[1] == 145 and params_maps.shape[-1] != 145:
        params_maps = params_maps.permute(0, 2, 3, 1)
    r, seen = _parse(center_maps, params_maps, centermap_parser.conf_thresh, centermap_parser.max_person,
                     watch=guard.watch if guard is not None else None)
    if guard is not None:
        rerun = guard.check(seen, next_in_flight=getattr(guard, 'pipelined', False))
        if r is None:
            if not (rerun and quiet):
                print('None person detected')
            return (None, None, rerun) if return_batch_ids else (None, rerun)
    elif r is None:
        print('None person detected')
        return (None, None) if return_batch_ids else None
    thetas = r['smpl_thetas']
    res = {
        'cam': r['cam'], 'global_orient': thetas[:, :3].contiguous(), 'body_pose': thetas[:, 3:].contiguous(),
        'smpl_betas': r['smpl_betas'], 'smpl_thetas': thetas,
        'center_preds': r['center_preds'], 'center_confs': r['scores'].unsqueeze(1),
    }
    if guard is not None:
        return (res, r['batch_ids'], rerun) if return_batch_ids else (res, rerun)
    return (res, r['batch_ids']) if return_batch_ids else res


def rot6D_to_angular(rot6D):
    lib = L.load()
    x = rot6D.contiguous().float()
    n = x.numel() // 6
    out = torch.empty(n, 3, device=x.device, dtype=torch.float32)
    with torch.cuda.device(x.device):
        L.check(lib.romp_rot6d_to_aa(L.ptr(x), n, L.ptr(out), L.stream_ptr(x.device)))
    return out.reshape(rot6D.shape[0], -1)


def convert_cam_to_3d_trans(cams, weight=2.):
    cams = cams.contiguous().float()
    out = torch.empty(cams.shape[0], 3, device=cams.device)
    with torch.cuda.device(cams.device):
        L.check(L.load().romp_cam_to_trans(L.ptr(cams), cams.shape[0], float(weight), L.ptr(out), L.stream_ptr(cams.device)))
    return out


try:
    import cv2 as _cv2
    _HAVE_CV2 = True
except Exception:
    _HAVE_CV2 = False


def estimate_translation_lsq(joints_3d, joints_2d, focal_length=443.4, img_size=(512., 512.)):
    X = np.asarray(joints_3d, np.float64)
    uv = np.asarray(joints_2d, np.float64)
    N = X.shape[0]
    f = float(focal_length)
    c = np.asarray(img_size, np.float64) / 2.
    w = ((np.asarray(joints_2d)[:, :, -1] > -2.) & (np.asarray(joints_3d)[:, :, -1] != -2.)).astype(np.float64)
    qx, qy = (c[0] - uv[:, :, 0]) * w, (c[1] - uv[:, :, 1]) * w
    rx = ((uv[:, :, 0] - c[0]) * X[:, :, 2] - f * X[:, :, 0]) * w
    ry = ((uv[:, :, 1] - c[1]) * X[:, :, 2] - f * X[:, :, 1]) * w
    out = np.full((N, 3), -1.0, np.float32)
    for i in range(N):
        d = w[i].sum() * f * f
        A = np.array([[d, 0, f * qx[i].sum()], [0, d, f * qy[i].sum()], [f * qx[i].sum(), f * qy[i].sum(), (qx[i] ** 2 + qy[i] ** 2).sum()]])
        b = np.array([f * rx[i].sum(), f * ry[i].sum(), (qx[i] * rx[i] + qy[i] * ry[i]).sum()])
        if w[i].sum() >= 4:
            try:
                out[i] = np.linalg.solve(A, b)
            except np.linalg.LinAlgError:
                pass
    return out


def pnp_translation(j24, p24):
    if not _HAVE_CV2:
        return None
    import cv2
    camK = np.eye(3)
    camK[0, 0] = camK[1, 1] = 443.4
    camK[:2, 2] = 256
    try:
        t = np.zeros((len(j24), 3), np.float32)
        for i in range(len(j24)):
            ret, rvec, tvec, inl = cv2.solvePnPRansac(j24[i], p24[i], camK, None, flags=cv2.SOLVEPNP_EPNP,
                                                      reprojectionError=20, iterationsCount=100)
            t[i] = -1 if inl is None else tvec[:, 0]
        return t
    except Exception:
        return None


def body_mesh_projection2image(j3d_preds, cam_preds, vertices=None, input2org_offsets=None, host_pnp=True):
    lib = L.load()
    dev = j3d_preds.device
    j = j3d_preds.contiguous().float()
    cam = cam_preds.contiguous().float()
    N, J = j.shape[:2]
    pad = input2org_offsets if input2org_offsets is not None else torch.tensor([0., 512., 0., 512., 512., 512.])
    pad_c = (C.c_float * 6)(*[float(v) for v in pad])
    pj2d = torch.empty(N, J, 2, device=dev)
    pj2d_org = torch.empty(N, J, 2, device=dev)
    ct = torch.empty(N, 3, device=dev)
    with torch.cuda.device(dev):
        L.check(lib.romp_project(L.ptr(j), N, J, L.ptr(cam), pad_c, L.ptr(pj2d), L.ptr(pj2d_org), L.ptr(ct),
                                 L.stream_ptr(dev)))
    trans = None
    if _HAVE_CV2 and host_pnp:
        t = pnp_translation(j[:, :24].detach().cpu().numpy(), (pj2d[:, :24].detach().cpu().numpy() + 1) * 256)
        trans = None if t is None else torch.from_numpy(t).float().to(dev)
    if trans is None:
        trans = torch.empty(N, 3, device=dev)
        with torch.cuda.device(dev):
            L.check(lib.romp_estimate_translation(L.ptr(j), N, J, 24, L.ptr(pj2d), 443.4, 512., L.ptr(trans), L.stream_ptr(dev)))
    out = {'pj2d': pj2d, 'cam_trans': trans}
    if input2org_offsets is not None:
        out['pj2d_org'] = pj2d_org
    if vertices is not None:
        v = vertices.contiguous().float()
        camed, org = torch.empty_like(v), torch.empty_like(v)
        with torch.cuda.device(dev):
            L.check(lib.romp_project_verts(L.ptr(v), v.shape[0], v.shape[1], L.ptr(cam), pad_c, L.ptr(camed), L.ptr(org), L.stream_ptr(dev)))
        out['verts_camed'] = camed
        if input2org_offsets is not None:
            out['verts_camed_org'] = org
    return out


class SMPL_parser(nn.Module):

    def __init__(self, model_path):
        super(SMPL_parser, self).__init__()
        self.smpl_model = SMPL(model_path)

    def forward(self, outputs, root_align=False):
        verts, joints, face = self.smpl_model(outputs['smpl_betas'], outputs['smpl_thetas'], root_align=root_align)
        outputs.update({'verts': verts, 'joints': joints, 'smpl_face': face})
        return outputs
```

Before: 3116 images/s.

## Fuse parse, pack, SMPL and record writes into one device-counted post pass

```diff
diff --git a/__graft_entry__.py b/__graft_entry__.py
--- a/__graft_entry__.py
+++ b/__graft_entry__.py
@@ -14,7 +14,7 @@
     import romp_amd
     from romp_amd import lib
     h = lib.load()
-    for name in lib.EXPORTS + lib.VIEW_EXPORTS:
+    for name in lib.EXPORTS + lib.VIEW_EXPORTS + lib.POST_EXPORTS:
         assert hasattr(h, name), name
     from oracle import romp_oracle
     if os.path.isdir('/root/reference/simple_romp/vis_human/sim3drender/lib'):
diff --git a/include/romp_hip_post.h b/include/romp_hip_post.h
--- /dev/null
+++ b/include/romp_hip_post.h
@@ -0,0 +1,35 @@
+#ifndef ROMP_HIP_POST_H
+#define ROMP_HIP_POST_H
+#include <stdint.h>
+#include "romp_hip.h"
+
+#ifdef __cplusplus
+extern "C" {
+#endif
+
+typedef struct romp_post_bufs {
+    float* cam;
+    float* smpl_thetas;
+    float* smpl_betas;
+    float* global_orient;
+    float* body_pose;
+    float* center_confs;
+    float* cam_trans;
+    int64_t* batch_ids;
+    int64_t* center_preds;
+    int32_t* flat_inds;
+    int32_t* count;
+    float* verts;
+    float* joints;
+    float* records;
+} romp_post_bufs;
+
+int romp_post_batch(const float* center_maps, const float* params_maps, int B, float conf_thresh, int max_person,
+                    smpl_ctx* smpl, int root_align, int with_joints, int with_verts, int64_t img_offset, int cap,
+                    const romp_post_bufs* bufs, int32_t* workspace, void* stream, const int32_t* watch,
+                    int32_t* count_host, int32_t* watch_host);
+
+#ifdef __cplusplus
+}
+#endif
+#endif
diff --git a/romp_amd/build.py b/romp_amd/build.py
--- a/romp_amd/build.py
+++ b/romp_amd/build.py
@@ -35,7 +35,7 @@
         with_bx3 = os.environ.get('ROMP_WITH_BX3', '0') not in ('', '0')
     sources = SOURCES + ([OPTIONAL_BX3] if with_bx3 else [])
     headers = [os.path.join(CSRC, f) for f in os.listdir(CSRC) if f.endswith('.h')] + \
-              [os.path.join(HERE, '..', 'include', h) for h in ('romp_hip.h', 'romp_hip_views.h')]
+              [os.path.join(HERE, '..', 'include', h) for h in ('romp_hip.h', 'romp_hip_views.h', 'romp_hip_post.h')]
     objdir = objdir or os.path.join(HERE, 'build')
     lib = lib or LIB
     os.makedirs(objdir, exist_ok=True)
diff --git a/romp_amd/csrc/common.h b/romp_amd/csrc/common.h
--- a/romp_amd/csrc/common.h
+++ b/romp_amd/csrc/common.h
@@ -64,6 +64,9 @@
 int launch_bev_pack(const float* fv, int fv_cs, const float* feats, int f_cs, float* out, int B, hipStream_t st);
 int launch_bev_maps(const float* fv, int fv_cs, const float* bv, int bv_cs, const float* anchors_host, float* center3d,
                     float* cam3d, int B, hipStream_t st);
+int smpl_forward_counted(smpl_ctx* c, const float* betas, const float* thetas, int cap, const int* n_dev, int root_align,
+                         float* verts, float* joints, hipStream_t st);
+
 int launch_conv3d(int C, const float* w_host, const float* scale_host, const float* shift_host, int relu, const float* in,
                   const float* res, float* out, int B, hipStream_t st);
 
diff --git a/romp_amd/csrc/parse.hip b/romp_amd/csrc/parse.hip
--- a/romp_amd/csrc/parse.hip
+++ b/romp_amd/csrc/parse.hip
@@ -1,5 +1,6 @@
 #include "common.h"
 #include "rot6d.h"
+#include "../../include/romp_hip_post.h"
 #include <vector>
 
 #pragma clang fp contract(off)
@@ -205,6 +206,84 @@
     org[i * 3 + 2] = (vz + 1.f) * pad_size / 2.f;
 }
 
+__global__ __launch_bounds__(64) void post_pack_kernel(const float* __restrict__ params, int B, int max_person, int cap,
+                                                       int32_t* __restrict__ ws, romp_post_bufs o, const int32_t* watch) {
+    const int r = blockIdx.x, b = blockIdx.y, lane = threadIdx.x;
+    const int stride = 2 * max_person + 2;
+    if (r == 0 && b == 0) {
+        if (watch && lane == 0)
+            ws[(size_t)B * stride] = __hip_atomic_load(watch, __ATOMIC_RELAXED, __HIP_MEMORY_SCOPE_AGENT);
+        int total = 0;
+        for (int k = lane; k < B; k += 64) total += ws[(size_t)k * stride + 2 * max_person];
+        for (int d = 32; d > 0; d >>= 1) total += __shfl_xor(total, d);
+        if (lane == 0) *o.count = total < cap ? total : cap;
+    }
+    const int cnt = ws[(size_t)b * stride + 2 * max_person];
+    if (r >= cnt) return;
+    int off = 0;
+    for (int k = lane; k < b; k += 64) off += ws[(size_t)k * stride + 2 * max_person];
+    for (int d = 32; d > 0; d >>= 1) off += __shfl_xor(off, d);
+    const int row = off + r;
+    if (row >= cap) return;
+    const int flat = ws[(size_t)b * stride + r];
+    const float sc = __int_as_float(ws[(size_t)b * stride + max_person + r]);
+    __shared__ float s_p[148];
+    const float* src = params + ((size_t)b * NPIX + flat) * 145;
+    for (int c = lane; c < 145; c += 64) {
+        float v = src[c];
+        if (c == 0) v = powf(1.1f, v);
+        s_p[c] = v;
+    }
+    __syncthreads();
+    if (lane < 3) o.cam[row * 3 + lane] = s_p[lane];
+    if (lane < 10) o.smpl_betas[row * 10 + lane] = s_p[135 + lane];
+    if (lane < 22) {
+        float aa[3];
+        rot6d_to_aa_dev(s_p + 3 + lane * 6, aa);
+        float* half = lane == 0 ? o.global_orient + (size_t)row * 3 : o.body_pose + (size_t)row * 69 + (lane - 1) * 3;
+        for (int k = 0; k < 3; ++k) {
+            o.smpl_thetas[(size_t)row * 72 + lane * 3 + k] = aa[k];
+            half[k] = aa[k];
+        }
+    } else if (lane < 28) {
+        o.smpl_thetas[(size_t)row * 72 + 66 + (lane - 22)] = 0.f;
+        o.body_pose[(size_t)row * 69 + 63 + (lane - 22)] = 0.f;
+    }
+    if (lane == 0) {
+        o.batch_ids[row] = b;
+        o.flat_inds[row] = flat;
+        o.center_confs[row] = sc;
+        o.center_preds[row * 2 + 0] = (flat % MAP) * 512 / 64;
+        o.center_preds[row * 2 + 1] = (flat / MAP) * 512 / 64;
+        const float s = s_p[0], tx = s_p[1], ty = s_p[2];
+        o.cam_trans[row * 3 + 0] = (tx / s) * 2.f;
+        o.cam_trans[row * 3 + 1] = (ty / s) * 2.f;
+        o.cam_trans[row * 3 + 2] = (1.f / s) * 2.f;
+    }
+}
+
+__global__ __launch_bounds__(256) void post_record_kernel(romp_post_bufs o, int with_joints, int with_verts, long long img_offset,
+                                                          int width) {
+    const int n = blockIdx.x, tid = threadIdx.x;
+    if (n >= *o.count) return;
+    float* d = o.records + (size_t)n * width;
+    if (tid == 0) {
+        d[0] = (float)(o.batch_ids[n] + img_offset);
+        d[1] = (float)o.flat_inds[n];
+        d[2] = o.center_confs[n];
+    }
+    if (tid < 3) d[3 + tid] = o.cam[n * 3 + tid];
+    if (tid < 72) d[6 + tid] = o.smpl_thetas[(size_t)n * 72 + tid];
+    if (tid < 10) d[78 + tid] = o.smpl_betas[n * 10 + tid];
+    int at = 88;
+    if (with_joints) {
+        if (tid < 213) d[at + tid] = o.joints[(size_t)n * 213 + tid];
+        at += 213;
+    }
+    if (with_verts)
+        for (int e = tid; e < 6890 * 3; e += 256) d[at + e] = o.verts[(size_t)n * 6890 * 3 + e];
+}
+
 }
 
 using namespace romp;
@@ -259,6 +338,41 @@
     return ROMP_OK;
 }
 
+int romp_post_batch(const float* center_maps, const float* params_maps, int B, float conf_thresh, int max_person,
+                    smpl_ctx* smpl, int root_align, int with_joints, int with_verts, int64_t img_offset, int cap,
+                    const romp_post_bufs* bufs, int32_t* workspace, void* stream, const int32_t* watch,
+                    int32_t* count_host, int32_t* watch_host) {
+    ROMP_REQUIRE(center_maps && params_maps && workspace && bufs && count_host && B > 0 && cap > 0, "romp_post_batch: bad arguments");
+    ROMP_REQUIRE(max_person >= 1 && max_person <= 1024, "romp_post_batch: max_person %d out of range", max_person);
+    const romp_post_bufs o = *bufs;
+    ROMP_REQUIRE(o.cam && o.smpl_thetas && o.smpl_betas && o.global_orient && o.body_pose && o.center_confs && o.cam_trans &&
+                 o.batch_ids && o.center_preds && o.flat_inds && o.count, "romp_post_batch: null output");
+    ROMP_REQUIRE(smpl ? (o.verts && o.joints) : (!with_joints && !with_verts), "romp_post_batch: meshes asked for without SMPL buffers");
+    hipStream_t st = (hipStream_t)stream;
+    hipLaunchKernelGGL(parse_nms_topk_kernel, dim3(B), dim3(PARSE_THREADS), 0, st, center_maps, conf_thresh, max_person, workspace);
+    ROMP_HIP_CHECK(hipGetLastError());
+    hipLaunchKernelGGL(post_pack_kernel, dim3(max_person, B), dim3(64), 0, st, params_maps, B, max_person, cap, workspace, o, watch);
+    ROMP_HIP_CHECK(hipGetLastError());
+    if (smpl) {
+        int rc = smpl_forward_counted(smpl, o.smpl_betas, o.smpl_thetas, cap, o.count, root_align, o.verts, o.joints, st);
+        if (rc) return rc;
+    }
+    if (o.records) {
+        const int width = 88 + (with_joints ? 213 : 0) + (with_verts ? 6890 * 3 : 0);
+        hipLaunchKernelGGL(post_record_kernel, dim3(cap), dim3(256), 0, st, o, with_joints, with_verts, (long long)img_offset, width);
+        ROMP_HIP_CHECK(hipGetLastError());
+    }
+    const size_t n_cnt = (size_t)B * (2 * max_person + 2);
+    std::vector<int32_t> cnt(n_cnt + 1);
+    ROMP_HIP_CHECK(hipMemcpyAsync(cnt.data(), workspace, (n_cnt + (watch ? 1 : 0)) * sizeof(int32_t), hipMemcpyDeviceToHost, st));
+    ROMP_HIP_CHECK(hipStreamSynchronize(st));
+    int total = 0;
+    for (int b = 0; b < B; ++b) total += cnt[(size_t)b * (2 * max_person + 2) + 2 * max_person];
+    *count_host = total;
+    if (watch && watch_host) *watch_host = cnt[n_cnt];
+    return ROMP_OK;
+}
+
 int romp_parse(const float* center_maps, const float* params_maps, int B, float conf_thresh, int max_person,
                int32_t* count_host, int32_t* batch_ids, int32_t* flat_inds, float* scores, float* params_pred,
                float* cam, float* thetas, float* betas, int32_t* center_preds, int32_t* workspace, void* stream) {
diff --git a/romp_amd/csrc/smpl.hip b/romp_amd/csrc/smpl.hip
--- a/romp_amd/csrc/smpl.hip
+++ b/romp_amd/csrc/smpl.hip
@@ -43,9 +43,11 @@
                                                         const float* __restrict__ thetas,
                                                         const float* __restrict__ Jt, const float* __restrict__ Js,
                                                         const int* __restrict__ sched, float* __restrict__ pose_feat,
-                                                        float* __restrict__ Amat, float* __restrict__ joints) {
+                                                        float* __restrict__ Amat, float* __restrict__ joints,
+                                                        const int* __restrict__ n_dev) {
     __shared__ float sR[NJ][9], sJ[NJ][3], sG[NJ][12];
     const int n = blockIdx.x, lane = threadIdx.x;
+    if (n_dev && n >= *n_dev) return;
     if (lane < NJ) {
         const float* r = thetas + (size_t)n * 72 + lane * 3;
         const float rx0 = r[0], ry0 = r[1], rz0 = r[2];
@@ -161,13 +163,19 @@
                                                          const float* __restrict__ Amat, const float* __restrict__ vt,
                                                          const float* __restrict__ sd, const float* __restrict__ pd,
                                                          const float* __restrict__ lbsw, const float* __restrict__ reg, int N, int groups,
-                                                         float* __restrict__ verts, float* __restrict__ jpart) {
+                                                         float* __restrict__ verts, float* __restrict__ jpart,
+                                                         const int* __restrict__ n_dev) {
     __shared__ __attribute__((aligned(16))) float s_u[U_FLOATS];
     __shared__ __attribute__((aligned(16))) float s_A[5 * 256 * 4];
     __shared__ float s_beta[PB][NB];
     static_assert(NPF * PB <= U_FLOATS && 4 * 256 * 4 <= U_FLOATS && PB * SVS <= U_FLOATS && NREG * RS <= PB * NJ * 12 && NT % 4 == 0, "LDS aliasing");
     const int tid = threadIdx.x, lane = tid & 63, wave = tid >> 6;
     const int xcd = blockIdx.x & 7, slot = blockIdx.x >> 3;
+    if (n_dev) {
+        N = *n_dev;
+        groups = (N + PB - 1) / PB;
+        if (groups == 0) return;
+    }
     const int tile = (slot / groups) * 8 + xcd, grp = slot % groups;
     if (tile >= NT) return;
     const int p0 = grp * PB;
@@ -307,9 +315,10 @@
 
 __global__ __launch_bounds__(256) void smpl_joints_kernel(const float* __restrict__ verts, const float* __restrict__ jpart,
                                                            const int* __restrict__ pick, int root_align, float* __restrict__ joints,
-                                                           float* __restrict__ root) {
+                                                           float* __restrict__ root, const int* __restrict__ n_dev) {
     __shared__ float s_j[NJOUT * 3];
     const int n = blockIdx.x, tid = threadIdx.x;
+    if (n_dev && n >= *n_dev) return;
     const float* vn = verts + (size_t)n * NV * 3;
     float* jn = joints + (size_t)n * NJOUT * 3;
     __shared__ float s_part[3][NREG * 3];
@@ -347,10 +356,11 @@
     }
 }
 
-__global__ __launch_bounds__(256) void smpl_root_sub_kernel(float* __restrict__ verts, const float* __restrict__ root) {
+__global__ __launch_bounds__(256) void smpl_root_sub_kernel(float* __restrict__ verts, const float* __restrict__ root,
+                                                             const int* __restrict__ n_dev) {
     const int n = blockIdx.y, i = blockIdx.x * 256 + threadIdx.x;
     static_assert(NV * 3 % 2 == 0, "person stride is a whole number of float2");
-    if (i >= NV * 3 / 2) return;
+    if (i >= NV * 3 / 2 || (n_dev && n >= *n_dev)) return;
     const float r0 = root[n * 3], r1 = root[n * 3 + 1], r2 = root[n * 3 + 2];
     float2* p = reinterpret_cast<float2*>(verts + (size_t)n * NV * 3) + i;
     float2 t = *p;
@@ -392,6 +402,42 @@
     ROMP_HIP_CHECK(hipMemsetAsync(c->Amat, 0, cap * NJ * 12 * 4, st));
     c->cap = (int)cap;
     return ROMP_OK;
+}
+
+static int smpl_launch(smpl_ctx* c, const float* betas, const float* thetas, int N, const int* n_dev, int root_align,
+                       float* verts, float* joints, hipStream_t st) {
+    int rc = smpl_reserve(c, N, st);
+    if (rc) return rc;
+    if (c->nb == 10)
+        hipLaunchKernelGGL(smpl_pose_kernel<10>, dim3(N), dim3(64), 0, st, betas, thetas, c->Jt, c->Js, c->sched, c->pose_feat, c->Amat, joints, n_dev);
+    else
+        hipLaunchKernelGGL(smpl_pose_kernel<11>, dim3(N), dim3(64), 0, st, betas, thetas, c->Jt, c->Js, c->sched, c->pose_feat, c->Amat, joints, n_dev);
+    ROMP_HIP_CHECK(hipGetLastError());
+    const int groups = (N + PB - 1) / PB;
+    const dim3 grid(8 * ((NT + 7) / 8) * groups);
+    if (c->nb == 10)
+        hipLaunchKernelGGL(smpl_skin_kernel<10>, grid, dim3(256), 0, st, betas, c->pose_feat, c->Amat, c->vt, c->sd, c->pd,
+                           c->lbsw, c->reg, N, groups, verts, c->jpart, n_dev);
+    else
+        hipLaunchKernelGGL(smpl_skin_kernel<11>, grid, dim3(256), 0, st, betas, c->pose_feat, c->Amat, c->vt, c->sd, c->pd,
+                           c->lbsw, c->reg, N, groups, verts, c->jpart, n_dev);
+    ROMP_HIP_CHECK(hipGetLastError());
+    hipLaunchKernelGGL(smpl_joints_kernel, dim3(N), dim3(256), 0, st, verts, c->jpart, c->pick, root_align, joints, c->root, n_dev);
+    ROMP_HIP_CHECK(hipGetLastError());
+    if (root_align) {
+        hipLaunchKernelGGL(smpl_root_sub_kernel, dim3((NV * 3 / 2 + 255) / 256, N), dim3(256), 0, st, verts, c->root, n_dev);
+        ROMP_HIP_CHECK(hipGetLastError());
+    }
+    return ROMP_OK;
+}
+
+namespace romp {
+int smpl_forward_counted(smpl_ctx* c, const float* betas, const float* thetas, int cap, const int* n_dev, int root_align,
+                         float* verts, float* joints, hipStream_t st) {
+    ROMP_REQUIRE(c && betas && thetas && verts && joints && n_dev && cap > 0, "smpl_forward_counted: bad arguments");
+    ROMP_REQUIRE(c->nb == 10, "smpl_forward_counted: the parameter rows of the parse carry 10 betas, the context has %d", c->nb);
+    return smpl_launch(c, betas, thetas, cap, n_dev, root_align, verts, joints, st);
+}
 }
 
 extern "C" {
@@ -480,30 +526,7 @@
     ROMP_REQUIRE(c && betas && thetas && verts && joints && N >= 0, "smpl_forward: bad arguments");
     ROMP_REQUIRE(n_betas == c->nb, "smpl_forward: n_betas %d but context was built with %d", n_betas, c->nb);
     if (N == 0) return ROMP_OK;
-    hipStream_t st = (hipStream_t)stream;
-    int rc = smpl_reserve(c, N, st);
-    if (rc) return rc;
-    if (c->nb == 10)
-        hipLaunchKernelGGL(smpl_pose_kernel<10>, dim3(N), dim3(64), 0, st, betas, thetas, c->Jt, c->Js, c->sched, c->pose_feat, c->Amat, joints);
-    else
-        hipLaunchKernelGGL(smpl_pose_kernel<11>, dim3(N), dim3(64), 0, st, betas, thetas, c->Jt, c->Js, c->sched, c->pose_feat, c->Amat, joints);
-    ROMP_HIP_CHECK(hipGetLastError());
-    const int groups = (N + PB - 1) / PB;
-    const dim3 grid(8 * ((NT + 7) / 8) * groups);
-    if (c->nb == 10)
-        hipLaunchKernelGGL(smpl_skin_kernel<10>, grid, dim3(256), 0, st, betas, c->pose_feat, c->Amat, c->vt, c->sd, c->pd,
-                           c->lbsw, c->reg, N, groups, verts, c->jpart);
-    else
-        hipLaunchKernelGGL(smpl_skin_kernel<11>, grid, dim3(256), 0, st, betas, c->pose_feat, c->Amat, c->vt, c->sd, c->pd,
-                           c->lbsw, c->reg, N, groups, verts, c->jpart);
-    ROMP_HIP_CHECK(hipGetLastError());
-    hipLaunchKernelGGL(smpl_joints_kernel, dim3(N), dim3(256), 0, st, verts, c->jpart, c->pick, root_align, joints, c->root);
-    ROMP_HIP_CHECK(hipGetLastError());
-    if (root_align) {
-        hipLaunchKernelGGL(smpl_root_sub_kernel, dim3((NV * 3 / 2 + 255) / 256, N), dim3(256), 0, st, verts, c->root);
-        ROMP_HIP_CHECK(hipGetLastError());
-    }
-    return ROMP_OK;
+    return smpl_launch(c, betas, thetas, N, nullptr, root_align, verts, joints, (hipStream_t)stream);
 }
 
 void smpl_ctx_destroy(smpl_ctx* c) {
diff --git a/romp_amd/distributed.py b/romp_amd/distributed.py
--- a/romp_amd/distributed.py
+++ b/romp_amd/distributed.py
@@ -23,6 +23,35 @@
     if with_verts:
         cols.append(outputs['verts'].reshape(N, -1))
     return torch.cat([c.to(dev).float() for c in cols], 1).contiguous()
+
+
+class RecordSink(object):
+
+    def __init__(self, device, img_offset, with_joints=False, with_verts=False, rows=0):
+        self.with_joints, self.with_verts, self.img_offset = bool(with_joints), bool(with_verts), int(img_offset)
+        self.width = record_width(with_joints, with_verts)
+        self.buf = torch.empty(int(rows), self.width, device=device, dtype=torch.float32)
+        self.n = 0
+
+    def room(self, cap):
+        if self.n + cap > self.buf.shape[0]:
+            grown = torch.empty(max(self.n + cap, 2 * self.buf.shape[0]), self.width, device=self.buf.device, dtype=torch.float32)
+            if self.n:
+                grown[:self.n] = self.buf[:self.n]
+            self.buf = grown
+        return self.buf[self.n:]
+
+    def took(self, n):
+        self.n += int(n)
+
+    def append(self, outputs, batch_ids, c0):
+        r = pack_records(outputs, batch_ids, self.img_offset + c0, with_joints=self.with_joints, with_verts=self.with_verts)
+        if r is not None:
+            self.room(r.shape[0])[:r.shape[0]] = r
+            self.n += r.shape[0]
+
+    def result(self):
+        return self.buf[:self.n] if self.n else None
 
 
 def record_width(with_joints=False, with_verts=False):
@@ -98,6 +127,13 @@
 def local_records(model, images_local, img_offset, chunk=None, with_joints=True, with_verts=False, next_images=None):
     n = images_local.shape[0]
     chunk = n if not chunk else int(chunk)
+    if chunk < n and getattr(model, 'packs_records', False) and (model.settings.calc_smpl or not (with_joints or with_verts)):
+        hint = model.__dict__.get('_record_rows', 0)
+        sink = RecordSink(images_local.device, img_offset, with_joints, with_verts, rows=hint)
+        for _ in model.forward_chunks(images_local, chunk, next_images=next_images, records=sink):
+            pass
+        model.__dict__['_record_rows'] = max(hint, sink.buf.shape[0])
+        return sink.result()
     recs = []
     if chunk < n and hasattr(model, 'forward_chunks'):
         it = model.forward_chunks(images_local, chunk, next_images=next_images) if next_images is not None else model.forward_chunks(images_local, chunk)
diff --git a/romp_amd/lib.py b/romp_amd/lib.py
--- a/romp_amd/lib.py
+++ b/romp_amd/lib.py
@@ -36,6 +36,11 @@
         ('weight', C.c_void_p), ('scale', C.c_void_p), ('shift', C.c_void_p), ('weight_aux', C.c_void_p),
         ('weight_h2', C.c_void_p), ('scale_h2', C.c_void_p),
     ]
+
+
+class RompPostBufs(C.Structure):
+    _fields_ = [(k, C.c_void_p) for k in ('cam', 'smpl_thetas', 'smpl_betas', 'global_orient', 'body_pose', 'center_confs', 'cam_trans',
+                                          'batch_ids', 'center_preds', 'flat_inds', 'count', 'verts', 'joints', 'records')]
 
 
 _lib = None
@@ -109,6 +114,8 @@
         'romp_bev_postprocess': (C.c_int, [vp, vp, vp, i32, vp, f, f, vp, vp, vp, vp, vp]),
         'romp_project': (C.c_int, [vp, i32, i32, vp, C.POINTER(C.c_float), vp, vp, vp, vp]),
         'romp_preprocess_crops': (C.c_int, [vp, i32, i32, i32, i32, C.POINTER(C.c_int32), vp, i32, C.POINTER(C.c_float), vp]),
+        'romp_post_batch': (C.c_int, [vp, vp, i32, f, i32, vp, i32, i32, i32, C.c_int64, i32, C.POINTER(RompPostBufs), vp, vp, vp,
+                                      C.POINTER(C.c_int32), C.POINTER(C.c_int32)]),
         'romp_bev_crowd_merge': (C.c_int, [vp, vp, vp, vp, i32, i32, i32, C.POINTER(C.c_int32), i32, i32, i32, C.c_double, f,
                                            vp, vp, vp, vp, vp, vp]),
     }
@@ -133,6 +140,7 @@
            'romp_project', 'romp_preprocess', 'romp_preprocess_batch', 'romp_bev_postprocess', 'romp_preprocess_crops',
            'romp_bev_crowd_merge']
 VIEW_EXPORTS = ['romp_sim3dr_render_batch', 'romp_view_weak_perspective']
+POST_EXPORTS = ['romp_post_batch']
 
 
 def has_bf16x3():
diff --git a/romp_amd/main.py b/romp_amd/main.py
--- a/romp_amd/main.py
+++ b/romp_amd/main.py
@@ -9,8 +9,8 @@
 
 from . import lib as L
 from .net import RangeGuard, RompNet
-from .post_parser import (_HAVE_CV2, CenterMap, SMPL_parser, body_mesh_projection2image, convert_cam_to_3d_trans, pnp_translation,
-                          parsing_outputs)
+from .post_parser import (_HAVE_CV2, CenterMap, PostBuffers, SMPL_parser, body_mesh_projection2image, convert_cam_to_3d_trans,
+                          pnp_translation, parsing_outputs, post_batch)
 from .vis import rendering_romp_bev_results, setup_renderer
 from .utils import ResultSaver, convert_tensor2numpy, determine_device, img_preprocess, img_preprocess_device
 
@@ -261,26 +261,66 @@
             outputs = rendering_romp_bev_results(self.renderer, outputs, image, rendering_cfgs)
         return convert_tensor2numpy(outputs)
 
+    packs_records = True
+
+    def _post_pass(self, center, params, pool_key=None, sink=None, c0=0, pipelined=False):
+        B = center.shape[0]
+        mp = self.centermap_parser.max_person
+        caps = self.__dict__.setdefault('_post_cap', {})
+        pool = self.__dict__.setdefault('_post_pool', {})
+        smpl = self.smpl_parser.smpl_model if self.settings.calc_smpl else None
+        while True:
+            cap = caps.setdefault(B, min(B * mp, max(64, 16 * B)))
+            pb = pool.get(pool_key) if pool_key is not None else None
+            if pb is None or pb.cap != cap or pb.B != B:
+                pb = PostBuffers(self.tdevice, cap, B, mp, smpl is not None)
+                if pool_key is not None:
+                    pool[pool_key] = pb
+            N, seen = post_batch(center, params, self.centermap_parser, pb, smpl_model=smpl, root_align=self.settings.root_align,
+                                 watch=self.range_guard.watch, records=sink.room(cap) if sink is not None else None,
+                                 with_joints=sink is not None and sink.with_joints, with_verts=sink is not None and sink.with_verts,
+                                 img_offset=(sink.img_offset + c0) if sink is not None else 0)
+            if N <= cap:
+                break
+            caps[B] = min(B * mp, (N * 5 // 4 + 15) // 16 * 16)
+        rerun = self.range_guard.check(seen, next_in_flight=pipelined)
+        if N == 0 or rerun:
+            if N == 0 and not rerun:
+                print('None person detected')
+            return None, None, rerun
+        if sink is not None:
+            sink.took(N)
+        v = pb.views
+        out = {k: v[k][:N] for k in ('cam', 'global_orient', 'body_pose', 'smpl_betas', 'smpl_thetas', 'center_preds', 'center_confs',
+                                     'cam_trans')}
+        if smpl is not None:
+            out.update({'verts': v['verts'][:N], 'joints': v['joints'][:N], 'smpl_face': smpl.faces_tensor})
+        return out, v['batch_ids'][:N], False
+
+    def _post_pass_f32(self, images):
+        c32, p32 = self._rerun_f32(images)
+        outputs, batch_ids = parsing_outputs(c32, p32, self.centermap_parser, return_batch_ids=True)
+        if outputs is not None:
+            outputs['cam_trans'] = convert_cam_to_3d_trans(outputs['cam'])
+            if self.settings.calc_smpl:
+                outputs = self.smpl_parser(outputs, root_align=self.settings.root_align)
+        return outputs, batch_ids
+
     @torch.no_grad()
     def forward_batch(self, images, return_tensors=True):
         center, params = self.model.forward_nhwc(images)
-        outputs, batch_ids, rerun = parsing_outputs(center.unsqueeze(1), params, self.centermap_parser, return_batch_ids=True,
-                                                    guard=self.range_guard, quiet=True)
+        outputs, batch_ids, rerun = self._post_pass(center, params)
         if rerun:
-            c32, p32 = self._rerun_f32(images)
-            outputs, batch_ids = parsing_outputs(c32, p32, self.centermap_parser, return_batch_ids=True)
+            outputs, batch_ids = self._post_pass_f32(images)
         if outputs is None:
             return None, None
-        outputs['cam_trans'] = convert_cam_to_3d_trans(outputs['cam'])
-        if self.settings.calc_smpl:
-            outputs = self.smpl_parser(outputs, root_align=self.settings.root_align)
         if not return_tensors:
             outputs = convert_tensor2numpy(outputs)
         return outputs, batch_ids
 
 
     @torch.no_grad()
-    def forward_chunks(self, images, chunk, next_images=None):
+    def forward_chunks(self, images, chunk, next_images=None, records=None):
         dev = self.tdevice
         n = images.shape[0]
         starts = list(range(0, n, chunk))
@@ -329,17 +369,12 @@
                 P['primed'] = dict(ptr=next_images.data_ptr(), shape=tuple(next_images.shape), chunk=chunk, par=par ^ 1,
                                    bufs=launch(next_images[:chunk], par ^ 1))
             cur.wait_event(P['ev_net'][par])
-            self.range_guard.pipelined = more or P['primed'] is not None
-            outputs, batch_ids, rerun = parsing_outputs(center.unsqueeze(1), params, self.centermap_parser, return_batch_ids=True,
-                                                        guard=self.range_guard, quiet=True)
-            self.range_guard.pipelined = False
+            outputs, batch_ids, rerun = self._post_pass(center, params, pool_key=(center.shape[0], par) if records is not None else None,
+                                                        sink=records, c0=c0, pipelined=more or P['primed'] is not None)
             if rerun:
-                c32, p32 = self._rerun_f32(images[c0:c0 + chunk])
-                outputs, batch_ids = parsing_outputs(c32, p32, self.centermap_parser, return_batch_ids=True)
-            if outputs is not None:
-                outputs['cam_trans'] = convert_cam_to_3d_trans(outputs['cam'])
-                if self.settings.calc_smpl:
-                    outputs = self.smpl_parser(outputs, root_align=self.settings.root_align)
+                outputs, batch_ids = self._post_pass_f32(images[c0:c0 + chunk])
+                if records is not None:
+                    records.append(outputs, batch_ids, c0)
             P['ev_free'][par].record(cur)
             yield outputs, batch_ids, c0
         if P['primed'] is None:
diff --git a/romp_amd/post_parser.py b/romp_amd/post_parser.py
--- a/romp_amd/post_parser.py
+++ b/romp_amd/post_parser.py
@@ -88,6 +88,50 @@
     return (res, r['batch_ids']) if return_batch_ids else res
 
 
+class PostBuffers(object):
+    F_COLS = (('cam', 3), ('smpl_thetas', 72), ('smpl_betas', 10), ('global_orient', 3), ('body_pose', 69), ('center_confs', 1),
+              ('cam_trans', 3))
+
+    def __init__(self, dev, cap, B, max_person, meshes):
+        self.cap, self.B, self.max_person = int(cap), int(B), int(max_person)
+        fbuf = torch.empty(cap * sum(w for _, w in self.F_COLS), device=dev, dtype=torch.float32)
+        v, at = {}, 0
+        for key, w in self.F_COLS:
+            v[key] = fbuf[at:at + cap * w].view(cap, w)
+            at += cap * w
+        lbuf = torch.empty(cap * 3, device=dev, dtype=torch.int64)
+        v['batch_ids'], v['center_preds'] = lbuf[:cap], lbuf[cap:].view(cap, 2)
+        ibuf = torch.empty(cap + 2 + B * (2 * max_person + 2) + 2, device=dev, dtype=torch.int32)
+        v['flat_inds'], self.count, self.ws = ibuf[:cap], ibuf[cap:cap + 1], ibuf[cap + 2:]
+        if meshes:
+            v['verts'] = torch.empty(cap, 6890, 3, device=dev, dtype=torch.float32)
+            v['joints'] = torch.empty(cap, 71, 3, device=dev, dtype=torch.float32)
+        self.views = v
+        self.c = L.RompPostBufs(**{k: v[k].data_ptr() for k in v}, count=self.count.data_ptr(), records=None)
+
+
+def post_batch(center_maps, params_maps_nhwc, centermap_parser, bufs, smpl_model=None, root_align=False, watch=None,
+               records=None, with_joints=False, with_verts=False, img_offset=0):
+    lib = L.load()
+    dev = center_maps.device
+    if dev.type != 'cuda':
+        raise L.RompHipError('parsing runs on the HIP device only (no CPU fallback)')
+    B = center_maps.shape[0]
+    cm = center_maps.reshape(B, 64, 64).contiguous().float()
+    pm = params_maps_nhwc.contiguous()
+    assert pm.shape == (B, 64, 64, 145) and pm.dtype == torch.float32 and B == bufs.B
+    if records is not None:
+        assert records.is_contiguous() and records.dtype == torch.float32 and records.shape[0] >= bufs.cap
+    bufs.c.records = records.data_ptr() if records is not None else None
+    n, w = C.c_int32(0), C.c_int32(0)
+    with torch.cuda.device(dev):
+        L.check(lib.romp_post_batch(L.ptr(cm), L.ptr(pm), B, float(centermap_parser.conf_thresh), int(centermap_parser.max_person),
+                                    smpl_model._context() if smpl_model is not None else None, int(bool(root_align)),
+                                    int(bool(with_joints)), int(bool(with_verts)), int(img_offset), bufs.cap, C.byref(bufs.c),
+                                    L.ptr(bufs.ws), L.stream_ptr(dev), C.c_void_p(watch or 0), C.byref(n), C.byref(w)))
+    return n.value, (w.value if watch else None)
+
+
 def rot6D_to_angular(rot6D):
     lib = L.load()
     x = rot6D.contiguous().float()
```

New measurement: 3103 images/s. Within noise of the previous version (-0.4%).
